# lfalive/fast-genomic-data-processing

Hardware: AMD Instinct MI355X
Metric: PairHMM GCUPS (higher is better)
Workload: dtype f32

## Files before the change

fast-genomic-data-processing_amd/csrc/mgx_pairhmm.hip:

```cpp
#include <hip/hip_runtime.h>

#include <algorithm>
#include <atomic>
#include <cerrno>
#include <cmath>
#include <cstdarg>
#include <cstdio>
#include <cstdlib>
#include <cstring>
#include <chrono>
#include <memory>
#include <mutex>
#include <new>
#include <thread>
#include <string>
#include <vector>

#include "../../include/mgx_pairhmm.h"
#include "mgx_common.h"
#include "mgx_tables.h"
#include "pairhmm_pack.h"
#include "pairhmm_kernels.hip.inc"

using mgx::set_error;

namespace {

constexpr int kNarrowMaxRPL = 8, kG8MaxRPL = 8, kG16MaxRPL = 12, kG64MinRPL = 4, kG64MaxRPL = 16;
constexpr int kMaxRowsG4 = 4 * kNarrowMaxRPL, kMaxRowsG8 = 8 * kG8MaxRPL;
constexpr int kMaxRowsG16 = 16 * kG16MaxRPL;
constexpr int kMaxRowsG64 = 64 * kG64MaxRPL;
constexpr int kMaxRowsStrip = 1 << 20;
constexpr int kStripMarkRPL = kG64MaxRPL + 1;
constexpr uint32_t kMaxLdsPerBlock = 64 * 1024;

struct Bin {
    int G = 0, RPL = 0;
    int Gd = 0, RPLd = 0;
    uint32_t job_begin = 0, job_count = 0;
    uint32_t max_h = 0;
    uint64_t cells = 0, alg_bytes = 0;
    uint32_t block = 256, lds_stride = 0, grid_f32 = 0, grid_f64 = 0, grid_f64_all = 0;
    bool strip = false;
};


struct Slab {
    uint8_t* dev = nullptr;
    uint8_t* pin = nullptr;
    size_t cap = 0, pin_cap = 0;
};
constexpr size_t kStageLimit = 256u << 20;
constexpr size_t kMaxEventSets = 64;
constexpr size_t kMinSlab = 1u << 20;
}

struct mgx_pairhmm {
    int device = 0;
    unsigned flags = 0;
    hipStream_t compute = nullptr, copy = nullptr, d2h = nullptr;
    static constexpr int kAux = 3;
    hipStream_t aux[kAux] = {nullptr, nullptr, nullptr};
    hipEvent_t ev_fork = nullptr, ev_join[kAux] = {nullptr, nullptr, nullptr};
    int n_streams = 1;
    float* d_ph2pr_f = nullptr; float* d_mm_f = nullptr; float* d_div3_f = nullptr; float* d_ratio_f = nullptr;
    double* d_ph2pr_d = nullptr; double* d_mm_d = nullptr; double* d_div3_d = nullptr; double* d_ratio_d = nullptr;
    float log10_initial_f = 0; double log10_initial_d = 0;
    int n_cu = 256;
    std::vector<Slab> free_slabs;
    void* d_strip = nullptr; size_t strip_cap = 0;
};

struct mgx_pairhmm_batch {
    uint64_t n_pairs = 0;
    std::vector<Bin> bins;
    Slab slab;
    size_t in_bytes = 0, o_out = 0, o_used = 0, result_bytes = 0;
    uint8_t *d_bases = nullptr, *d_qual = nullptr, *d_ins = nullptr, *d_del = nullptr,
            *d_gcp = nullptr, *d_hap = nullptr, *d_used = nullptr;
    Job* d_jobs = nullptr;
    uint32_t* d_rerun_list = nullptr;
    uint32_t* d_rerun_count = nullptr;
    double* d_out = nullptr;
    std::vector<Job> host_jobs;
    bool has_model = false;
    uint32_t n_reads = 0;
    uint64_t* d_read_len = nullptr;
    uint8_t* d_keep = nullptr;
    uint32_t *d_row_off = nullptr, *d_row_nh = nullptr;
    size_t o_keep = 0;
    double log10_rate = 0, max_err = 0;
    hipEvent_t uploaded = nullptr;
    std::vector<hipEvent_t> ev;
    std::vector<uint64_t> acct_cells, acct_bytes;
    std::vector<int8_t> acct_multi;
    uint32_t ev_sets = 0;
    uint32_t runs_timed = 0;
    hipEvent_t done = nullptr;
    bool ran = false;
    mgx_pairhmm_stats_t stats{};
};

namespace {

using BatchPtr = std::unique_ptr<mgx_pairhmm_batch, void (*)(mgx_pairhmm_batch*)>;
BatchPtr new_batch() {
    return BatchPtr(new (std::nothrow) mgx_pairhmm_batch, [](mgx_pairhmm_batch* p) { mgx_pairhmm_batch_destroy(nullptr, p); });
}

#define HIP_TRY(expr)                                                                      \
    do {                                                                                   \
        hipError_t e_ = (expr);                                                            \
        if (e_ != hipSuccess) {                                                            \
            set_error("%s failed: %s (%s:%d)", #expr, hipGetErrorString(e_), __FILE__,     \
                      __LINE__);                                                           \
            return -EIO;                                                                   \
        }                                                                                  \
    } while (0)

template <typename T>
int upload(T** dst, const void* src, size_t bytes, hipStream_t s) {
    *dst = nullptr;
    if (bytes == 0) bytes = 16;
    HIP_TRY(hipMalloc((void**)dst, bytes));
    if (src) HIP_TRY(hipMemcpyAsync(*dst, src, bytes, hipMemcpyHostToDevice, s));
    return 0;
}

inline void shape_of(uint32_t R, int* G, int* RPL) {
    static const int min_g = [] { const char* e = getenv("MGX_PAIRHMM_MIN_G"); const int v = e ? atoi(e) : 4; return v; }();
    const uint32_t g8_rows = (uint32_t)kMaxRowsG8;
    if (R <= (uint32_t)kMaxRowsG4 && min_g <= 4) { *G = 4; *RPL = (int)((R + 3) / 4); }
    else if (R <= g8_rows && min_g <= 8) { *G = 8; *RPL = (int)((R + 7) / 8); }
    else if (R <= (uint32_t)kMaxRowsG16) { *G = 16; *RPL = (int)((R + 15) / 16); }
    else if (R <= (uint32_t)kMaxRowsG64) { *G = 64; *RPL = std::max(kG64MinRPL, (int)((R + 63) / 64)); }
    else if (R <= (uint32_t)kMaxRowsStrip) { *G = 64; *RPL = kStripMarkRPL; }
    else { *G = 0; *RPL = 0; }
}
inline uint32_t lds_bytes(const Bin& bin, bool f32) {
    const uint32_t waves = bin.block / 64u, groups = bin.block / (uint32_t)(f32 ? bin.G : bin.Gd);
    const uint32_t etab = f32 ? (uint32_t)((bin.RPL + 1) / 2) * kNumCodes * 512u : 0u;
    return waves * etab + groups * bin.lds_stride;
}
constexpr int kBinG8 = kNarrowMaxRPL, kBinG16 = kBinG8 + kG8MaxRPL, kBinG64 = kBinG16 + kG16MaxRPL;
constexpr int kBinStrip = kBinG64 + (kG64MaxRPL - kG64MinRPL + 1);
constexpr int kBins = kBinStrip + 1;
inline int bin_index(int G, int RPL) {
    if (G == 64 && RPL == kStripMarkRPL) return kBinStrip;
    return G == 4 ? RPL - 1 : G == 8 ? kBinG8 + RPL - 1 : G == 16 ? kBinG16 + RPL - 1 : kBinG64 + RPL - kG64MinRPL;
}
inline void bin_shape(int k, Bin* b) {
    if (k == kBinStrip) { b->G = 64; b->RPL = kG64MaxRPL; b->Gd = 64; b->RPLd = kG64MaxRPL; b->strip = true; return; }
    if (k < kBinG8) { b->G = 4; b->RPL = k + 1; }
    else if (k < kBinG16) { b->G = 8; b->RPL = k - kBinG8 + 1; }
    else if (k < kBinG64) { b->G = 16; b->RPL = k - kBinG16 + 1; }
    else { b->G = 64; b->RPL = k - kBinG64 + kG64MinRPL; }
    if (b->G == 16 && b->RPL > 8) { b->Gd = 64; b->RPLd = (16 * b->RPL + 63) / 64; }
    else { b->Gd = b->G; b->RPLd = b->RPL; }
}
constexpr uint64_t kMergeBelow = 4096;

int finalize_bin(Bin& bin, int n_cu) {
    bin.lds_stride = (bin.max_h + 2u * (uint32_t)std::max(bin.G, bin.Gd) + 8u + 15u) & ~15u;
    bin.block = 64;
    if (const char* e = getenv("MGX_PAIRHMM_BLOCK")) { const int v = atoi(e); if (v == 64 || v == 128 || v == 256) bin.block = (uint32_t)v; }
    while (bin.block > 64u && lds_bytes(bin, true) > kMaxLdsPerBlock) bin.block /= 2;
    if (lds_bytes(bin, true) > 160u * 1024u) {
        set_error("haplotype of %u bases does not fit the LDS staging buffer", bin.max_h);
        return -E2BIG;
    }
    if (bin.strip) {
        bin.block = 64;
        bin.grid_f32 = bin.grid_f64 = bin.grid_f64_all = std::min<uint32_t>(bin.job_count, (uint32_t)n_cu * 4u);
        return 0;
    }
    const uint32_t gpb = bin.block / bin.G, gpbd = bin.block / bin.Gd;
    bin.grid_f32 = (bin.job_count + gpb - 1) / gpb;
    bin.grid_f64_all = (bin.job_count + gpbd - 1) / gpbd;
    bin.grid_f64 = std::min<uint32_t>(bin.grid_f64_all, (uint32_t)n_cu * 8u);
    return 0;
}
void merge_small_bins(uint64_t (&count)[kBins], int (&remap)[kBins]) {
    for (int k = 0; k < kBins; ++k) remap[k] = k;
    for (int k = 0; k + 1 < kBins; ++k) {
        if (k + 1 == kBinG8 || k + 1 == kBinG16 || k + 1 == kBinG64 || k + 1 == kBinStrip) continue;
        if (count[k] && count[k] < kMergeBelow) { count[k + 1] += count[k]; count[k] = 0; remap[k] = k + 1; }
    }
    for (int k = 0; k < kBins; ++k) { int t = k; while (remap[t] != t) t = remap[t]; remap[k] = t; }
}

inline size_t align_up(size_t x, size_t a = 256) { return (x + a - 1) / a * a; }

int acquire_slab(mgx_pairhmm* c, size_t bytes, size_t pin_bytes, Slab* out) {
    int best = -1;
    for (size_t i = 0; i < c->free_slabs.size(); ++i) {
        const Slab& f = c->free_slabs[i];
        if (f.cap >= bytes && f.pin_cap >= pin_bytes && (best < 0 || f.cap < c->free_slabs[best].cap)) best = (int)i;
    }
    if (best >= 0) { *out = c->free_slabs[best]; c->free_slabs.erase(c->free_slabs.begin() + best); return 0; }
    auto round = [](size_t want) {
        size_t cap = kMinSlab;
        while (cap < want) cap *= 2;
        if (cap > want + (want >> 2) && want > (64u << 20)) cap = align_up(want, 1u << 20);
        return cap;
    };
    Slab sl;
    sl.cap = round(bytes);
    HIP_TRY(hipMalloc((void**)&sl.dev, sl.cap));
    if (pin_bytes) {
        sl.pin_cap = std::min(sl.cap, round(pin_bytes));
        if (hipHostMalloc((void**)&sl.pin, sl.pin_cap, hipHostMallocDefault) != hipSuccess) {
            (void)hipFree(sl.dev);
            set_error("hipHostMalloc of %zu bytes failed", sl.pin_cap);
            return -ENOMEM;
        }
    }
    *out = sl;
    return 0;
}
void release_slab(mgx_pairhmm* c, Slab sl) {
    if (!sl.dev) return;
    if (c && c->free_slabs.size() < 16) { c->free_slabs.push_back(sl); return; }
    (void)hipFree(sl.dev);
    if (sl.pin) (void)hipHostFree(sl.pin);
}

using mgx::validate;

}

extern "C" {

int mgx_pairhmm_table_f32(int which, const float** out) {
    const auto& t = mgx::tables<float>();
    if (which == 0) { *out = t.ph2pr.data(); return mgx::kPh2prSize; }
    if (which == 1) { *out = t.mm.data(); return mgx::kMmSize; }
    return -EINVAL;
}
int mgx_pairhmm_table_f64(int which, const double** out) {
    const auto& t = mgx::tables<double>();
    if (which == 0) { *out = t.ph2pr.data(); return mgx::kPh2prSize; }
    if (which == 1) { *out = t.mm.data(); return mgx::kMmSize; }
    return -EINVAL;
}

int mgx_pairhmm_create(int device, unsigned flags, mgx_pairhmm_t** out) {
    if (!out) { set_error("out is NULL"); return -EINVAL; }
    *out = nullptr;
    int n_dev = 0;
    if (hipGetDeviceCount(&n_dev) != hipSuccess || n_dev <= 0) {
        set_error("no HIP device is visible (this library has no CPU fallback)");
        return -ENODEV;
    }
    if (device == -1) {
        static std::atomic<unsigned> next{0};
        device = (int)(next.fetch_add(1) % (unsigned)n_dev);
    }
    if (device < 0 || device >= n_dev) { set_error("device %d out of range (0..%d)", device, n_dev - 1); return -EINVAL; }
    HIP_TRY(hipSetDevice(device));
    std::unique_ptr<mgx_pairhmm> c(new (std::nothrow) mgx_pairhmm);
    if (!c) return -ENOMEM;
    c->device = device;
    c->flags = flags;
    hipDeviceProp_t prop;
    HIP_TRY(hipGetDeviceProperties(&prop, device));
    c->n_cu = prop.multiProcessorCount;
    {
        const unsigned pat = (flags >> 8) & 0xFFu;
        if (pat != 0 && pat != 0xFFu) {
            const int n_words = (c->n_cu + 31) / 32;
            std::vector<uint32_t> mask(n_words, 0);
            for (int cu = 0; cu < c->n_cu; ++cu) if ((pat >> (cu & 7)) & 1u) mask[cu >> 5] |= 1u << (cu & 31);
            HIP_TRY(hipExtStreamCreateWithCUMask(&c->compute, (uint32_t)n_words, mask.data()));
        } else {
            HIP_TRY(hipStreamCreateWithFlags(&c->compute, hipStreamNonBlocking));
        }
    }
    HIP_TRY(hipStreamCreateWithFlags(&c->copy, hipStreamNonBlocking));
    HIP_TRY(hipStreamCreateWithFlags(&c->d2h, hipStreamNonBlocking));
    {
        const unsigned pat = (flags >> 8) & 0xFFu;
        const char* e = getenv("MGX_PAIRHMM_STREAMS");
        c->n_streams = e ? std::max(1, std::min(1 + mgx_pairhmm::kAux, atoi(e))) : 1;
        if (pat != 0 && pat != 0xFFu) c->n_streams = 1;
        for (int a = 0; a + 1 < c->n_streams; ++a) {
            HIP_TRY(hipStreamCreateWithFlags(&c->aux[a], hipStreamNonBlocking));
            HIP_TRY(hipEventCreateWithFlags(&c->ev_join[a], hipEventDisableTiming));
        }
        HIP_TRY(hipEventCreateWithFlags(&c->ev_fork, hipEventDisableTiming));
    }
    const auto& tf = mgx::tables<float>();
    const auto& td = mgx::tables<double>();
    int rc;
    if ((rc = upload(&c->d_ph2pr_f, tf.ph2pr.data(), tf.ph2pr.size() * 4, c->compute))) return rc;
    if ((rc = upload(&c->d_mm_f, tf.mm.data(), tf.mm.size() * 4, c->compute))) return rc;
    if ((rc = upload(&c->d_ph2pr_d, td.ph2pr.data(), td.ph2pr.size() * 8, c->compute))) return rc;
    if ((rc = upload(&c->d_mm_d, td.mm.data(), td.mm.size() * 8, c->compute))) return rc;
    if ((rc = upload(&c->d_div3_f, tf.ph2pr_div3.data(), tf.ph2pr_div3.size() * 4, c->compute))) return rc;
    if ((rc = upload(&c->d_ratio_f, tf.gap_ratio.data(), tf.gap_ratio.size() * 4, c->compute))) return rc;
    if ((rc = upload(&c->d_div3_d, td.ph2pr_div3.data(), td.ph2pr_div3.size() * 8, c->compute))) return rc;
    if ((rc = upload(&c->d_ratio_d, td.gap_ratio.data(), td.gap_ratio.size() * 8, c->compute))) return rc;
    c->log10_initial_f = tf.log10_initial;
    c->log10_initial_d = td.log10_initial;
    HIP_TRY(hipStreamSynchronize(c->compute));
    *out = c.release();
    return 0;
}

void mgx_pairhmm_destroy(mgx_pairhmm_t* c) {
    if (!c) return;
    (void)hipSetDevice(c->device);
    (void)hipFree(c->d_ph2pr_f); (void)hipFree(c->d_mm_f);
    (void)hipFree(c->d_ph2pr_d); (void)hipFree(c->d_mm_d);
    (void)hipFree(c->d_div3_f); (void)hipFree(c->d_ratio_f); (void)hipFree(c->d_div3_d); (void)hipFree(c->d_ratio_d);
    for (auto& sl : c->free_slabs) { (void)hipFree(sl.dev); if (sl.pin) (void)hipHostFree(sl.pin); }
    (void)hipFree(c->d_strip);
    if (c->compute) (void)hipStreamDestroy(c->compute);
    if (c->copy) (void)hipStreamDestroy(c->copy);
    if (c->d2h) (void)hipStreamDestroy(c->d2h);
    for (int a = 0; a < mgx_pairhmm::kAux; ++a) { if (c->aux[a]) (void)hipStreamDestroy(c->aux[a]); if (c->ev_join[a]) (void)hipEventDestroy(c->ev_join[a]); }
    if (c->ev_fork) (void)hipEventDestroy(c->ev_fork);
    delete c;
}

void mgx_pairhmm_batch_destroy(mgx_pairhmm_t* c, mgx_pairhmm_batch_t* b) {
    if (!b) return;
    if (c) {
        (void)hipSetDevice(c->device);
        if (b->done) (void)hipEventSynchronize(b->done);
        else if (b->uploaded) (void)hipEventSynchronize(b->uploaded);
    }
    release_slab(c, b->slab);
    if (b->uploaded) (void)hipEventDestroy(b->uploaded);
    if (b->done) (void)hipEventDestroy(b->done);
    for (auto e : b->ev) (void)hipEventDestroy(e);
    delete b;
}

namespace {

struct SlabLayout {
    uint64_t n = 0, n_reads = 0, n_haps = 0, n_regions = 0, read_bytes = 0, hap_bytes = 0;
    bool cross = false, model = false;
    size_t rtab = 0, rreg = 0, rpre = 0, gtab = 0, htab = 0;
    size_t jobs = 0, bases = 0, qual = 0, ins = 0, del = 0, gcp = 0, hap = 0;
    size_t mapq = 0, rlen = 0, roff = 0, rnh = 0;
    size_t rlist = 0, rcount = 0;
    size_t pin_bytes = 0;
    bool staged = true;
};

int lay_out_slab(mgx_pairhmm* c, bool always_stage, SlabLayout* L, mgx_pairhmm_batch* b) {
    size_t off = 0;
    auto take = [&off](size_t bytes) { const size_t at = off; off = align_up(off + bytes); return at; };
    const uint64_t n = L->n, per_read = L->model ? L->n_reads : 0;
    if (L->cross) {
        L->rtab = take(L->n_reads * sizeof(SeqRef));
        L->rreg = take(L->n_reads * sizeof(uint32_t));
        L->rpre = take((L->n_reads + 1) * sizeof(uint32_t));
        L->gtab = take(L->n_regions * sizeof(RegionRef));
        L->htab = take(L->n_haps * sizeof(SeqRef));
    } else {
        L->jobs = take(n * sizeof(Job));
    }
    L->bases = take(L->read_bytes);
    L->qual = take(L->read_bytes);
    L->ins = take(L->read_bytes);
    L->del = take(L->read_bytes);
    L->gcp = take(L->read_bytes);
    L->hap = take(L->hap_bytes);
    L->mapq = take(per_read);
    L->rlen = take(per_read * sizeof(uint64_t));
    L->roff = take(per_read * sizeof(uint32_t));
    L->rnh = take(per_read * sizeof(uint32_t));
    b->in_bytes = off;
    b->o_out = take(n * sizeof(double));
    b->o_used = take(n);
    b->o_keep = take(per_read);
    b->result_bytes = off - b->o_out;
    L->pin_bytes = off;
    if (L->cross) L->jobs = take(n * sizeof(Job));
    L->rlist = take(2 * n * sizeof(uint32_t));
    L->rcount = take(64 * sizeof(uint32_t));
    L->staged = always_stage || L->pin_bytes <= kStageLimit;
    if (const int rc = acquire_slab(c, off, L->staged ? L->pin_bytes : 0, &b->slab)) return rc;
    uint8_t* dv = b->slab.dev;
    b->d_jobs = (Job*)(dv + L->jobs);
    b->d_bases = dv + L->bases; b->d_qual = dv + L->qual; b->d_ins = dv + L->ins; b->d_del = dv + L->del;
    b->d_gcp = dv + L->gcp; b->d_hap = dv + L->hap;
    b->d_out = (double*)(dv + b->o_out); b->d_used = dv + b->o_used;
    b->d_rerun_list = (uint32_t*)(dv + L->rlist); b->d_rerun_count = (uint32_t*)(dv + L->rcount);
    if (L->model) {
        b->d_read_len = (uint64_t*)(dv + L->rlen); b->d_keep = dv + b->o_keep;
        b->d_row_off = (uint32_t*)(dv + L->roff); b->d_row_nh = (uint32_t*)(dv + L->rnh);
    }
    return 0;
}

ReadModel make_read_model(const mgx_read_model_t& model) {
    ReadModel rm{};
    rm.rate_factor = model.pcr_rate_factor; rm.bq_threshold = model.base_quality_threshold;
    rm.constant_gcp = model.constant_gcp;
    for (int i = 0; i <= 20; ++i) {
        const double d = 40.0 - std::exp((double)i / ((double)std::max(rm.rate_factor, 1) * M_PI));
        const int v = (d > 0.0 ? (int)(d + 0.5) : (int)(d - 0.5)) + 1;
        rm.pcr_cache[i] = (uint8_t)(char)std::max(10, v);
    }
    return rm;
}

struct CrossRead { uint64_t off; uint32_t len, region; uint8_t bin; };
struct CrossPlan {
    uint64_t nr = 0, nh = 0, n = 0, read_bytes = 0, hap_bytes = 0;
    std::vector<CrossRead> reads;
    std::vector<RegionRef> regions;
    std::vector<SeqRef> haps;
    uint32_t max_h = 0;
    uint64_t reads_in[kBins] = {0}, rstart[kBins + 1] = {0}, jobs_in[kBins] = {0}, cells_in[kBins] = {0}, bytes_in[kBins] = {0};
};

int cross_totals(uint32_t n_regions, const mgx_pairhmm_input_t* regs, CrossPlan* p, std::vector<uint64_t>* out_base) {
    out_base->assign(n_regions + 1, 0);
    for (uint32_t g = 0; g < n_regions; ++g) {
        const mgx_pairhmm_input_t& in = regs[g];
        if (in.pair_read || in.pair_hap) { set_error("region %u: regions are given in the cross-product form (pair arrays NULL)", g); return -EINVAL; }
        p->nr += in.n_reads; p->nh += in.n_haps; p->n += in.n_reads * in.n_haps;
        if (in.n_reads) p->read_bytes += in.read_off[in.n_reads] - in.read_off[0];
        if (in.n_haps) p->hap_bytes += in.hap_off[in.n_haps] - in.hap_off[0];
        (*out_base)[g + 1] = p->n;
    }
    if (p->n > 0xFFFFFFF0ull || p->nr > 0xFFFFFFF0ull) { set_error("more than 2^32 test cases in one batch"); return -E2BIG; }
    return 0;
}

int cross_tables(uint32_t n_regions, const mgx_pairhmm_input_t* regs, const std::vector<uint64_t>& out_base, CrossPlan* p,
                 uint64_t (&count)[kBins]) {
    p->reads.resize(p->nr); p->regions.resize(n_regions); p->haps.resize(p->nh);
    uint64_t r_at = 0, h_at = 0, rb = 0, hb = 0;
    for (uint32_t g = 0; g < n_regions; ++g) {
        const mgx_pairhmm_input_t& in = regs[g];
        RegionRef& R = p->regions[g];
        R.hap_begin = (uint32_t)h_at; R.n_haps = (uint32_t)in.n_haps; R.read_base = (uint32_t)r_at; R.out_base = (uint32_t)out_base[g];
        for (uint64_t h = 0; h < in.n_haps; ++h) {
            const uint64_t H = in.hap_off[h + 1] - in.hap_off[h];
            if (H == 0) { set_error("region %u: haplotype %llu is empty", g, (unsigned long long)h); return -EINVAL; }
            if (H > 0x7FFFFFF0ull) { set_error("haplotype too long"); return -E2BIG; }
            p->haps[h_at + h] = SeqRef{hb + (in.hap_off[h] - in.hap_off[0]), (uint32_t)H, (uint32_t)h};
            p->max_h = std::max<uint32_t>(p->max_h, (uint32_t)H);
        }
        std::stable_sort(p->haps.begin() + h_at, p->haps.begin() + h_at + in.n_haps, [](const SeqRef& a, const SeqRef& b2) { return a.len > b2.len; });
        for (uint64_t r = 0; r < in.n_reads; ++r) {
            const uint64_t Rl = in.read_off[r + 1] - in.read_off[r];
            if (Rl == 0) { set_error("region %u: read %llu is empty", g, (unsigned long long)r); return -EINVAL; }
            int G, RPL;
            shape_of((uint32_t)std::min<uint64_t>(Rl, 0xFFFFFFFFull), &G, &RPL);
            if (G == 0) { set_error("region %u: read of %llu bases exceeds the %d-row limit", g, (unsigned long long)Rl, kMaxRowsStrip); return -E2BIG; }
            CrossRead& ri = p->reads[r_at + r];
            ri.off = rb + (in.read_off[r] - in.read_off[0]); ri.len = (uint32_t)Rl; ri.region = g; ri.bin = (uint8_t)bin_index(G, RPL);
            count[ri.bin] += in.n_haps;
        }
        if (in.n_reads) rb += in.read_off[in.n_reads] - in.read_off[0];
        if (in.n_haps) hb += in.hap_off[in.n_haps] - in.hap_off[0];
        r_at += in.n_reads; h_at += in.n_haps;
    }
    return 0;
}

void cross_bins(CrossPlan* p, uint64_t (&count)[kBins]) {
    int remap[kBins];
    merge_small_bins(count, remap);
    std::vector<uint64_t> sumH(p->regions.size(), 0);
    for (size_t g = 0; g < p->regions.size(); ++g)
        for (uint32_t h = 0; h < p->regions[g].n_haps; ++h) sumH[g] += p->haps[p->regions[g].hap_begin + h].len;
    for (CrossRead& ri : p->reads) {
        ri.bin = (uint8_t)remap[ri.bin];
        const RegionRef& R = p->regions[ri.region];
        p->reads_in[ri.bin]++; p->jobs_in[ri.bin] += R.n_haps; p->cells_in[ri.bin] += (uint64_t)ri.len * sumH[ri.region];
        p->bytes_in[ri.bin] += 5ull * ri.len * R.n_haps + sumH[ri.region] + 4ull * R.n_haps;
    }
    for (int k = 0; k < kBins; ++k) p->rstart[k + 1] = p->rstart[k] + p->reads_in[k];
}

void cross_stage(const CrossPlan& p, uint32_t n_regions, const mgx_pairhmm_input_t* regs, const SlabLayout& L, uint8_t* pin) {
    SeqRef* rtab = (SeqRef*)(pin + L.rtab);
    uint32_t* rreg = (uint32_t*)(pin + L.rreg);
    uint32_t* rpre = (uint32_t*)(pin + L.rpre);
    uint64_t cur[kBins];
    for (int k = 0; k < kBins; ++k) cur[k] = p.rstart[k];
    for (uint64_t r = 0; r < p.nr; ++r) {
        const CrossRead& ri = p.reads[r];
        const uint64_t at = cur[ri.bin]++;
        rtab[at] = SeqRef{ri.off, ri.len, (uint32_t)r};
        rreg[at] = ri.region;
    }
    uint32_t run = 0;
    for (uint64_t at = 0; at < p.nr; ++at) { rpre[at] = run; run += p.regions[rreg[at]].n_haps; }
    rpre[p.nr] = run;
    memcpy(pin + L.gtab, p.regions.data(), n_regions * sizeof(RegionRef));
    memcpy(pin + L.htab, p.haps.data(), p.nh * sizeof(SeqRef));
    size_t rb = 0, hb = 0;
    for (uint32_t g = 0; g < n_regions; ++g) {
        const mgx_pairhmm_input_t& in = regs[g];
        if (in.n_reads) {
            const uint64_t o0 = in.read_off[0], len = in.read_off[in.n_reads] - o0;
            memcpy(pin + L.bases + rb, in.bases + o0, len); memcpy(pin + L.qual + rb, in.qual + o0, len);
            memcpy(pin + L.ins + rb, in.ins + o0, len);     memcpy(pin + L.del + rb, in.del + o0, len);
            memcpy(pin + L.gcp + rb, in.gcp + o0, len);
            rb += len;
        }
        if (in.n_haps) {
            const uint64_t o0 = in.hap_off[0], len = in.hap_off[in.n_haps] - o0;
            memcpy(pin + L.hap + hb, in.hap_bases + o0, len);
            hb += len;
        }
    }
}

int cross_stage_model(uint32_t n_regions, const mgx_pairhmm_input_t* regs, const uint8_t* const* mapq,
                      const std::vector<uint64_t>& out_base, const SlabLayout& L, uint8_t* pin) {
    uint64_t* rlen = (uint64_t*)(pin + L.rlen);
    uint32_t* roff = (uint32_t*)(pin + L.roff);
    uint32_t* rnh = (uint32_t*)(pin + L.rnh);
    uint64_t r_at = 0;
    for (uint32_t g = 0; g < n_regions; ++g) {
        const mgx_pairhmm_input_t& in = regs[g];
        if (in.n_reads && !mapq[g]) { set_error("region %u: mapq is NULL", g); return -EINVAL; }
        for (uint64_t r = 0; r < in.n_reads; ++r) {
            rlen[r_at + r] = in.read_off[r + 1] - in.read_off[r];
            roff[r_at + r] = (uint32_t)(out_base[g] + r * in.n_haps);
            rnh[r_at + r] = (uint32_t)in.n_haps;
        }
        if (in.n_reads) memcpy(pin + L.mapq + r_at, mapq[g], in.n_reads);
        r_at += in.n_reads;
    }
    return 0;
}

int create_cross(mgx_pairhmm_t* c, uint32_t n_regions, const mgx_pairhmm_input_t* regs, mgx_pairhmm_batch* b,
                 std::vector<uint64_t>* out_base, const uint8_t* const* mapq = nullptr, const mgx_read_model_t* model = nullptr) {
    CrossPlan p;
    int rc;
    if ((rc = cross_totals(n_regions, regs, &p, out_base))) return rc;
    b->n_pairs = p.n;
    b->stats.n_pairs = p.n;
    if (p.n == 0) return 0;
    uint64_t count[kBins] = {0};
    if ((rc = cross_tables(n_regions, regs, *out_base, &p, count))) return rc;
    cross_bins(&p, count);
    SlabLayout L;
    L.n = p.n; L.n_reads = p.nr; L.n_haps = p.nh; L.n_regions = n_regions; L.read_bytes = p.read_bytes; L.hap_bytes = p.hap_bytes;
    L.cross = true; L.model = model != nullptr;
    if ((rc = lay_out_slab(c, true, &L, b))) return rc;
    uint8_t* dv = b->slab.dev; uint8_t* pin = b->slab.pin;
    cross_stage(p, n_regions, regs, L, pin);
    hipStream_t s = c->copy;
    if (model) {
        if ((rc = cross_stage_model(n_regions, regs, mapq, *out_base, L, pin))) return rc;
        b->has_model = true; b->n_reads = (uint32_t)p.nr;
        b->log10_rate = model->log10_mismapping_rate; b->max_err = model->max_error_per_base;
    }
    HIP_TRY(hipMemcpyAsync(dv, pin, b->in_bytes, hipMemcpyHostToDevice, s));
    if (model)
        hipLaunchKernelGGL(pairhmm_read_model, dim3((uint32_t)p.nr), dim3(128), 0, s, (const SeqRef*)(dv + L.rtab),
                           b->d_bases, b->d_qual, b->d_ins, b->d_del, b->d_gcp, (const uint8_t*)(dv + L.mapq), make_read_model(*model));
    uint64_t job_begin = 0;
    for (int k = 0; k < kBins; ++k) {
        if (!p.reads_in[k]) continue;
        Bin bin;
        bin_shape(k, &bin);
        bin.job_begin = (uint32_t)job_begin;
        bin.job_count = (uint32_t)p.jobs_in[k];
        bin.max_h = p.max_h;
        bin.cells = p.cells_in[k];
        bin.alg_bytes = p.bytes_in[k];
        if ((rc = finalize_bin(bin, c->n_cu))) return rc;
        b->stats.cells += bin.cells; b->stats.alg_bytes += bin.alg_bytes;
        b->bins.push_back(bin);
        job_begin += bin.job_count;
    }
    hipLaunchKernelGGL(pairhmm_make_jobs_multi, dim3((uint32_t)((p.n + 255) / 256)), dim3(256), 0, s, (const SeqRef*)(dv + L.rtab),
                       (const uint32_t*)(dv + L.rreg), (const uint32_t*)(dv + L.rpre), (uint32_t)p.nr, (const RegionRef*)(dv + L.gtab),
                       (const SeqRef*)(dv + L.htab), (uint32_t)p.n, b->d_jobs);
    HIP_TRY(hipGetLastError());
    HIP_TRY(hipEventCreateWithFlags(&b->uploaded, hipEventDisableTiming));
    HIP_TRY(hipEventRecord(b->uploaded, s));
    return 0;
}

int upload_pairs(mgx_pairhmm_t* c, const mgx_pairhmm_input_t* in, const mgx::PackPlan* plan, const SlabLayout& L, const Job* jobs,
                 mgx_pairhmm_batch* b) {
    const uint64_t read_bytes = L.read_bytes, hap_bytes = L.hap_bytes;
    uint8_t* dv = b->slab.dev;
    hipStream_t s = c->copy;
    if (L.staged) {
        uint8_t* pin = b->slab.pin;
        if (plan) {
            mgx::pack_copy(in, *plan, pin + L.bases, pin + L.qual, pin + L.ins, pin + L.del, pin + L.gcp, pin + L.hap);
        } else if (read_bytes + hap_bytes < (32u << 20)) {
            memcpy(pin + L.bases, in->bases, read_bytes); memcpy(pin + L.qual, in->qual, read_bytes);
            memcpy(pin + L.ins, in->ins, read_bytes);     memcpy(pin + L.del, in->del, read_bytes);
            memcpy(pin + L.gcp, in->gcp, read_bytes);     memcpy(pin + L.hap, in->hap_bases, hap_bytes);
        } else {
            const void* src[6] = {in->bases, in->qual, in->ins, in->del, in->gcp, in->hap_bases};
            uint8_t* dst[6] = {pin + L.bases, pin + L.qual, pin + L.ins, pin + L.del, pin + L.gcp, pin + L.hap};
            const size_t len[6] = {(size_t)read_bytes, (size_t)read_bytes, (size_t)read_bytes, (size_t)read_bytes, (size_t)read_bytes, (size_t)hap_bytes};
            std::thread th[6];
            for (int k = 0; k < 6; ++k) th[k] = std::thread([=] { memcpy(dst[k], src[k], len[k]); });
            for (auto& t : th) t.join();
        }
        HIP_TRY(hipMemcpyAsync(dv, pin, b->in_bytes, hipMemcpyHostToDevice, s));
    } else {
        HIP_TRY(hipMemcpyAsync(b->d_jobs, jobs, L.n * sizeof(Job), hipMemcpyHostToDevice, s));
        HIP_TRY(hipMemcpyAsync(b->d_bases, in->bases, read_bytes, hipMemcpyHostToDevice, s));
        HIP_TRY(hipMemcpyAsync(b->d_qual, in->qual, read_bytes, hipMemcpyHostToDevice, s));
        HIP_TRY(hipMemcpyAsync(b->d_ins, in->ins, read_bytes, hipMemcpyHostToDevice, s));
        HIP_TRY(hipMemcpyAsync(b->d_del, in->del, read_bytes, hipMemcpyHostToDevice, s));
        HIP_TRY(hipMemcpyAsync(b->d_gcp, in->gcp, read_bytes, hipMemcpyHostToDevice, s));
        HIP_TRY(hipMemcpyAsync(b->d_hap, in->hap_bases, hap_bytes, hipMemcpyHostToDevice, s));
        HIP_TRY(hipStreamSynchronize(s));
        b->host_jobs.clear(); b->host_jobs.shrink_to_fit();
    }
    HIP_TRY(hipEventCreateWithFlags(&b->uploaded, hipEventDisableTiming));
    HIP_TRY(hipEventRecord(b->uploaded, s));
    return 0;
}

int create_pairs(mgx_pairhmm_t* c, const mgx_pairhmm_input_t* in, const mgx::PackPlan* plan, mgx_pairhmm_batch* b) {
    const uint64_t n = plan ? plan->hi - plan->lo : in->n_pairs;
    const uint32_t* pr = plan ? plan->pair_read.data() : in->pair_read;
    const uint32_t* ph = plan ? plan->pair_hap.data() : in->pair_hap;
    const uint64_t* roff = plan ? plan->roff.data() : in->read_off;
    const uint64_t* hoff = plan ? plan->hoff.data() : in->hap_off;
    const uint64_t n_reads = plan ? plan->lread.size() : in->n_reads, n_haps = plan ? plan->lhap.size() : in->n_haps;
    int rc;
    b->n_pairs = n;
    b->stats.n_pairs = n;

    std::vector<uint32_t> bin_of(n);
    uint64_t count[kBins] = {0};
    uint32_t max_h = 0;
    for (uint64_t i = 0; i < n; ++i) {
        const uint32_t r = pr[i], h = ph[i];
        if (r >= n_reads || h >= n_haps) { set_error("test case %llu: index out of range", (unsigned long long)i); return -EINVAL; }
        const uint64_t R = roff[r + 1] - roff[r];
        const uint64_t H = hoff[h + 1] - hoff[h];
        if (R == 0 || H == 0) { set_error("test case %llu: empty read or haplotype", (unsigned long long)i); return -EINVAL; }
        int G, RPL;
        shape_of((uint32_t)std::min<uint64_t>(R, 0xFFFFFFFFull), &G, &RPL);
        if (G == 0) { set_error("test case %llu: read of %llu bases exceeds the %d-row limit", (unsigned long long)i, (unsigned long long)R, kMaxRowsStrip); return -E2BIG; }
        if (H > 0x7FFFFFF0ull) { set_error("haplotype too long"); return -E2BIG; }
        const int bi = bin_index(G, RPL);
        bin_of[i] = (uint32_t)bi;
        count[bi]++;
        max_h = std::max<uint32_t>(max_h, (uint32_t)H);
        b->stats.cells += R * H;
        b->stats.alg_bytes += 5 * R + H + 4;
    }
    {
        int remap[kBins];
        merge_small_bins(count, remap);
        for (uint64_t i = 0; i < n; ++i) bin_of[i] = (uint32_t)remap[bin_of[i]];
    }
    SlabLayout L;
    L.n = n; L.n_reads = n_reads; L.n_haps = n_haps; L.read_bytes = roff[n_reads]; L.hap_bytes = hoff[n_haps];
    if ((rc = lay_out_slab(c, plan != nullptr, &L, b))) return rc;
    if (!L.staged) b->host_jobs.resize(n);
    Job* jobs = L.staged ? (Job*)(b->slab.pin + L.jobs) : b->host_jobs.data();
    {
        std::vector<uint64_t> bin_start(kBins + 1, 0);
        for (int k = 0; k < kBins; ++k) bin_start[k + 1] = bin_start[k] + count[k];
        std::vector<std::vector<uint32_t>> hist(kBins);
        for (int k = 0; k < kBins; ++k) if (count[k]) hist[k].assign((size_t)max_h + 2, 0);
        for (uint64_t i = 0; i < n; ++i) {
            const uint32_t h = ph[i];
            const uint32_t H = (uint32_t)(hoff[h + 1] - hoff[h]);
            hist[bin_of[i]][(max_h - H) + 1]++;
        }
        for (int k = 0; k < kBins; ++k)
            for (size_t x = 1; x < hist[k].size(); ++x) hist[k][x] += hist[k][x - 1];
        for (uint64_t i = 0; i < n; ++i) {
            const uint32_t r = pr[i], h = ph[i];
            const uint32_t R = (uint32_t)(roff[r + 1] - roff[r]);
            const uint32_t H = (uint32_t)(hoff[h + 1] - hoff[h]);
            const int k = (int)bin_of[i];
            Job& jb = jobs[bin_start[k] + hist[k][max_h - H]++];
            jb.read_off = roff[r]; jb.hap_off = hoff[h];
            jb.R = R; jb.H = H; jb.pair = (uint32_t)i; jb.pad_ = 0;
        }
        for (int k = 0; k < kBins; ++k) {
            if (!count[k]) continue;
            Bin bin;
            bin_shape(k, &bin);
            bin.job_begin = (uint32_t)bin_start[k];
            bin.job_count = (uint32_t)count[k];
            for (uint64_t q = bin_start[k]; q < bin_start[k + 1]; ++q) {
                bin.max_h = std::max(bin.max_h, jobs[q].H);
                bin.cells += (uint64_t)jobs[q].R * jobs[q].H;
                bin.alg_bytes += 5ull * jobs[q].R + jobs[q].H + 4;
            }
            if ((rc = finalize_bin(bin, c->n_cu))) return rc;
            b->bins.push_back(bin);
        }
    }
    return upload_pairs(c, in, plan, L, jobs, b);
}

}

int mgx_pairhmm_batch_create(mgx_pairhmm_t* c, const mgx_pairhmm_input_t* in,
                             mgx_pairhmm_batch_t** out) {
    if (!c || !out) { set_error("ctx/out is NULL"); return -EINVAL; }
    *out = nullptr;
    int rc = validate(in);
    if (rc) return rc;
    HIP_TRY(hipSetDevice(c->device));
    BatchPtr b = new_batch();
    if (!b) return -ENOMEM;
    std::vector<uint64_t> base;
    if (!in->pair_read && !in->pair_hap && in->n_reads && in->n_haps) rc = create_cross(c, 1, in, b.get(), &base);
    else rc = create_pairs(c, in, nullptr, b.get());
    if (rc) return rc;
    *out = b.release();
    return 0;
}

namespace {

constexpr int kSharedCount = 63;
constexpr int kExactCount = 62;

inline bool is_narrow(const Bin& bn) { return bn.G <= 16 && bn.G * bn.RPL <= 16 * kNarrowMaxRPL; }

struct Run {
    mgx_pairhmm* c = nullptr;
    mgx_pairhmm_batch* b = nullptr;
    hipStream_t s = nullptr;
    bool timing = false, force_f64 = false;
    hipEvent_t* ev = nullptr;
    int n_str = 1;
    KernelArgs base{};
    std::vector<char> in_multi;
    size_t first_narrow = 0;
    uint32_t n_narrow_jobs = 0, narrow_max_h = 0, narrow_rows = 0;
};

int ensure_strip_scratch(mgx_pairhmm* c, size_t bytes) {
    if (bytes <= c->strip_cap) return 0;
    HIP_TRY(hipStreamSynchronize(c->compute));
    (void)hipFree(c->d_strip); c->d_strip = nullptr; c->strip_cap = 0;
    HIP_TRY(hipMalloc(&c->d_strip, bytes));
    c->strip_cap = bytes;
    return 0;
}

int pick_event_set(Run& r) {
    mgx_pairhmm_batch* b = r.b;
    if (!r.timing) return 0;
    if (b->ev.empty()) {
        const size_t per = b->bins.size() * 4;
        b->ev_sets = (uint32_t)std::max<size_t>(1, std::min<size_t>(kMaxEventSets, 1024 / per));
        b->ev.resize(per * b->ev_sets);
        for (auto& e : b->ev) HIP_TRY(hipEventCreate(&e));
    }
    r.ev = b->ev.data() + (size_t)(b->runs_timed % b->ev_sets) * b->bins.size() * 4;
    return 0;
}

int begin_run(Run& r) {
    mgx_pairhmm* c = r.c; mgx_pairhmm_batch* b = r.b;
    if (b->uploaded) HIP_TRY(hipStreamWaitEvent(r.s, b->uploaded, 0));
    HIP_TRY(hipMemsetAsync(b->d_rerun_count, 0, 64 * sizeof(uint32_t), r.s));
    HIP_TRY(hipMemsetAsync(b->d_used, 0, b->n_pairs, r.s));
    r.n_str = (int)std::min<size_t>((size_t)c->n_streams, b->bins.size());
    if (r.n_str > 1) {
        HIP_TRY(hipEventRecord(c->ev_fork, r.s));
        for (int q = 0; q + 1 < r.n_str; ++q) HIP_TRY(hipStreamWaitEvent(c->aux[q], c->ev_fork, 0));
    }
    KernelArgs& base = r.base;
    base.jobs = b->d_jobs;
    base.bases = b->d_bases; base.qual = b->d_qual; base.ins = b->d_ins; base.del = b->d_del;
    base.gcp = b->d_gcp; base.hap_bases = b->d_hap;
    base.out_log10 = b->d_out; base.used_f64 = b->d_used;
    base.log10_initial_f = c->log10_initial_f;
    base.log10_initial_d = c->log10_initial_d;
    return 0;
}

void survey_narrow(Run& r) {
    const std::vector<Bin>& bins = r.b->bins;
    r.first_narrow = bins.size();
    for (size_t k = 0; k < bins.size(); ++k) {
        const Bin& bn = bins[k];
        if (!is_narrow(bn)) continue;
        if (r.first_narrow == bins.size()) r.first_narrow = k;
        r.n_narrow_jobs = std::max(r.n_narrow_jobs, bn.job_begin + bn.job_count);
        r.narrow_max_h = std::max(r.narrow_max_h, bn.max_h);
        r.narrow_rows = std::max(r.narrow_rows, (uint32_t)(bn.G * bn.RPL));
    }
}

int launch_f64(const Run& r, KernelArgs a, int Gd, int RPLd, uint32_t grid, uint32_t block, uint32_t lds, hipStream_t sk) {
    const mgx_pairhmm* c = r.c;
    a.ph2pr = c->d_ph2pr_d; a.mm = c->d_mm_d; a.ph2pr_div3 = c->d_div3_d; a.gap_ratio = c->d_ratio_d;
    a.rerun_list = r.b->d_rerun_list + r.b->n_pairs; a.rerun_count = r.b->d_rerun_count + kExactCount;
    KernelFn f = a.strip_scratch ? (KernelFn)pairhmm_fwd_strip<double> : pick_kernel<double>(Gd, RPLd);
    if (!f) { set_error("no fp64 kernel for G=%d RPL=%d", Gd, RPLd); return -ENOSYS; }
    hipLaunchKernelGGL(f, dim3(grid), dim3(block), lds, sk, a);
    return 0;
}

int launch_multi(Run& r, int gset, std::vector<size_t>& set) {
    mgx_pairhmm* c = r.c; mgx_pairhmm_batch* b = r.b;
    std::stable_sort(set.begin(), set.end(), [&](size_t x, size_t y) {
        const Bin &bx = b->bins[x], &by = b->bins[y];
        return bx.RPL != by.RPL ? bx.RPL > by.RPL : bx.G > by.G;
    });
    MultiArgs m{};
    m.a = r.base;
    m.a.rerun_list = b->d_rerun_list; m.a.rerun_count = b->d_rerun_count + kSharedCount;
    m.a.job_list = nullptr; m.a.n_dyn = nullptr;
    m.a.ph2pr = c->d_ph2pr_f; m.a.mm = c->d_mm_f; m.a.ph2pr_div3 = c->d_div3_f; m.a.gap_ratio = c->d_ratio_f;
    m.n_bins = (uint32_t)set.size();
    uint32_t blocks = 0, lds = 0;
    size_t book = set[0];
    uint64_t cells = 0, bytes = 0;
    for (size_t q = 0; q < set.size(); ++q) {
        const Bin& bn = b->bins[set[q]];
        m.block_first[q] = blocks; blocks += bn.grid_f32;
        m.job_first[q] = bn.job_begin; m.job_count[q] = bn.job_count; m.lds_stride[q] = bn.lds_stride;
        m.G[q] = (uint8_t)bn.G; m.RPL[q] = (uint8_t)bn.RPL;
        lds = std::max(lds, lds_bytes(bn, true));
        if (bn.cells > b->bins[book].cells) book = set[q];
        cells += bn.cells; bytes += bn.alg_bytes;
        r.in_multi[set[q]] = 1;
        b->acct_cells[set[q]] = 0; b->acct_bytes[set[q]] = 0;
    }
    m.block_first[set.size()] = blocks;
    b->acct_cells[book] = cells; b->acct_bytes[book] = bytes; b->acct_multi[book] = (int8_t)(1 + gset);
    if (r.timing) for (size_t q : set) if (q != book) { HIP_TRY(hipEventRecord(r.ev[4 * q + 0], r.s)); HIP_TRY(hipEventRecord(r.ev[4 * q + 1], r.s)); }
    if (r.timing) HIP_TRY(hipEventRecord(r.ev[4 * book + 0], r.s));
    if (gset == 0) hipLaunchKernelGGL(pairhmm_fwd_multi<0>, dim3(blocks), dim3(64), lds, r.s, m);
    else           hipLaunchKernelGGL(pairhmm_fwd_multi<1>, dim3(blocks), dim3(64), lds, r.s, m);
    if (r.timing) HIP_TRY(hipEventRecord(r.ev[4 * book + 1], r.s));
    return 0;
}

int launch_multi_classes(Run& r) {
    mgx_pairhmm_batch* b = r.b;
    static const bool multi_ok = [] { const char* e = getenv("MGX_PAIRHMM_MULTI"); return !e || atoi(e) != 0; }();
    const uint32_t multi_below = (uint32_t)r.c->n_cu * 64u;
    r.in_multi.assign(b->bins.size(), 0);
    b->acct_cells.assign(b->bins.size(), 0); b->acct_bytes.assign(b->bins.size(), 0); b->acct_multi.assign(b->bins.size(), 0);
    for (size_t k = 0; k < b->bins.size(); ++k) { b->acct_cells[k] = b->bins[k].cells; b->acct_bytes[k] = b->bins[k].alg_bytes; }
    if (!multi_ok || r.force_f64) return 0;
    for (int gset = 0; gset < 2; ++gset) {
        std::vector<size_t> set;
        for (size_t k = 0; k < b->bins.size(); ++k) {
            const Bin& bn = b->bins[k];
            if (is_narrow(bn) && bn.RPL <= kNarrowMaxRPL && bn.block == 64 && bn.grid_f32 < multi_below && (gset == 0 ? bn.G == 16 : bn.G < 16)) set.push_back(k);
        }
        if (set.size() < 2 || set.size() > (size_t)kMultiBins) continue;
        if (const int rc = launch_multi(r, gset, set)) return rc;
    }
    return 0;
}

int launch_class(Run& r, size_t k, hipStream_t sk) {
    mgx_pairhmm* c = r.c; mgx_pairhmm_batch* b = r.b;
    hipEvent_t* ev = r.ev;
    const Bin& bin = b->bins[k];
    const bool shared = is_narrow(bin) && !r.force_f64;
    KernelArgs a = r.base;
    if (bin.strip) {
        a.strip_stride = (bin.max_h + 63u) & ~63u;
        if (const int rc = ensure_strip_scratch(c, (size_t)bin.grid_f32 * 6u * a.strip_stride * sizeof(double))) return rc;
        a.strip_scratch = c->d_strip;
    }
    a.rerun_list = shared ? b->d_rerun_list : b->d_rerun_list + bin.job_begin;
    a.rerun_count = b->d_rerun_count + (shared ? kSharedCount : (int)k);
    a.lds_stride = bin.lds_stride;
    a.job_first = bin.job_begin;
    if (!r.force_f64 && !r.in_multi[k]) {
        a.job_list = nullptr; a.n_dyn = nullptr; a.n_static = bin.job_count;
        a.ph2pr = c->d_ph2pr_f; a.mm = c->d_mm_f; a.ph2pr_div3 = c->d_div3_f; a.gap_ratio = c->d_ratio_f;
        KernelFn f = bin.strip ? (KernelFn)pairhmm_fwd_strip<float> : pick_kernel<float>(bin.G, bin.RPL);
        if (!f) { set_error("no fp32 kernel for G=%d RPL=%d", bin.G, bin.RPL); return -ENOSYS; }
        if (r.timing) HIP_TRY(hipEventRecord(ev[4 * k + 0], sk));
        hipLaunchKernelGGL(f, dim3(bin.grid_f32), dim3(bin.block), lds_bytes(bin, true), sk, a);
        if (r.timing) HIP_TRY(hipEventRecord(ev[4 * k + 1], sk));
    }
    const bool books_shared = shared && k == r.first_narrow;
    if (r.timing && !books_shared) HIP_TRY(hipEventRecord(ev[4 * k + 2], sk));
    if (!shared) {
        if (r.force_f64) { a.job_list = nullptr; a.n_dyn = nullptr; a.n_static = bin.job_count; }
        else { a.job_list = a.rerun_list; a.n_dyn = a.rerun_count; a.n_static = 0; }
        const int rc = launch_f64(r, a, bin.Gd, bin.RPLd, r.force_f64 ? bin.grid_f64_all : bin.grid_f64, bin.block, lds_bytes(bin, false), sk);
        if (rc) return rc;
    }
    if (r.timing && !books_shared) HIP_TRY(hipEventRecord(ev[4 * k + 3], sk));
    return 0;
}

int launch_classes(Run& r) {
    mgx_pairhmm* c = r.c; mgx_pairhmm_batch* b = r.b;
    std::vector<size_t> order(b->bins.size());
    for (size_t k = 0; k < order.size(); ++k) order[k] = k;
    std::stable_sort(order.begin(), order.end(), [&](size_t x, size_t y) { return b->bins[x].cells > b->bins[y].cells; });
    for (size_t at = 0; at < order.size(); ++at) {
        hipStream_t sk = (int)(at % (size_t)r.n_str) == 0 ? r.s : c->aux[at % (size_t)r.n_str - 1];
        if (const int rc = launch_class(r, order[at], sk)) return rc;
    }
    for (int q = 0; q + 1 < r.n_str; ++q) {
        HIP_TRY(hipEventRecord(c->ev_join[q], c->aux[q]));
        HIP_TRY(hipStreamWaitEvent(r.s, c->ev_join[q], 0));
    }
    return 0;
}

int launch_shared_f64(Run& r) {
    if (!r.n_narrow_jobs || r.force_f64) return 0;
    KernelArgs a = r.base;
    a.job_list = r.b->d_rerun_list; a.n_dyn = r.b->d_rerun_count + kSharedCount; a.n_static = 0; a.job_first = 0;
    a.lds_stride = (r.narrow_max_h + 2u * 16u + 8u + 15u) & ~15u;
    const int RPLd = (int)((r.narrow_rows + 15) / 16);
    const uint32_t grid = std::min<uint32_t>((r.n_narrow_jobs + 3) / 4, (uint32_t)r.c->n_cu * 8u);
    if (r.timing) HIP_TRY(hipEventRecord(r.ev[4 * r.first_narrow + 2], r.s));
    if (const int rc = launch_f64(r, a, 16, RPLd, grid, 64, 4u * a.lds_stride, r.s)) return rc;
    if (r.timing) HIP_TRY(hipEventRecord(r.ev[4 * r.first_narrow + 3], r.s));
    return 0;
}

int launch_exact(Run& r) {
    mgx_pairhmm* c = r.c; mgx_pairhmm_batch* b = r.b;
    uint32_t max_h = 0;
    for (const Bin& bn : b->bins) max_h = std::max(max_h, bn.max_h);
    KernelArgs a = r.base;
    a.ph2pr = c->d_ph2pr_d; a.mm = c->d_mm_d; a.ph2pr_div3 = c->d_div3_d; a.gap_ratio = c->d_ratio_d;
    a.job_list = b->d_rerun_list + b->n_pairs; a.n_dyn = b->d_rerun_count + kExactCount; a.n_static = 0; a.job_first = 0;
    a.rerun_list = nullptr; a.rerun_count = nullptr;
    a.lds_stride = (max_h + 2u * 64u + 8u + 15u) & ~15u;
    a.strip_stride = (max_h + 63u) & ~63u;
    const size_t per_wg = 6u * (size_t)a.strip_stride * sizeof(double);
    const uint32_t grid = (uint32_t)std::max<size_t>(1, std::min<size_t>({(size_t)b->n_pairs, (size_t)c->n_cu * 2u, (size_t)(256u << 20) / per_wg}));
    if (const int rc = ensure_strip_scratch(c, (size_t)grid * per_wg)) return rc;
    a.strip_scratch = c->d_strip;
    hipLaunchKernelGGL(pairhmm_fwd_exact, dim3(grid), dim3(64), a.lds_stride, r.s, a);
    return 0;
}

void launch_epilogue(Run& r) {
    const mgx_pairhmm_batch* b = r.b;
    if (!b->has_model) return;
    hipLaunchKernelGGL(pairhmm_normalize_filter_rows, dim3((b->n_reads + 3) / 4), dim3(256), 0, r.s, b->d_out, b->d_read_len,
                       b->d_row_off, b->d_row_nh, b->n_reads, b->log10_rate, b->max_err, b->d_keep);
}

}

int mgx_pairhmm_batch_run(mgx_pairhmm_t* c, mgx_pairhmm_batch_t* b) {
    if (!c || !b) { set_error("ctx/batch is NULL"); return -EINVAL; }
    HIP_TRY(hipSetDevice(c->device));
    if (b->n_pairs == 0) { b->ran = true; return 0; }
    Run r;
    r.c = c; r.b = b; r.s = c->compute;
    r.timing = (c->flags & MGX_PAIRHMM_TIMING) != 0 && !b->bins.empty();
    r.force_f64 = (c->flags & MGX_PAIRHMM_FORCE_DOUBLE) != 0;
    int rc;
    if ((rc = pick_event_set(r))) return rc;
    if ((rc = begin_run(r))) return rc;
    survey_narrow(r);
    if ((rc = launch_multi_classes(r))) return rc;
    if ((rc = launch_classes(r))) return rc;
    if ((rc = launch_shared_f64(r))) return rc;
    if ((rc = launch_exact(r))) return rc;
    launch_epilogue(r);
    HIP_TRY(hipGetLastError());
    if (r.timing) b->runs_timed++;
    if (!b->done) HIP_TRY(hipEventCreateWithFlags(&b->done, hipEventDisableTiming));
    HIP_TRY(hipEventRecord(b->done, r.s));
    b->ran = true;
    return 0;
}

int mgx_pairhmm_sync(mgx_pairhmm_t* c) {
    if (!c) { set_error("ctx is NULL"); return -EINVAL; }
    HIP_TRY(hipSetDevice(c->device));
    HIP_TRY(hipStreamSynchronize(c->compute));
    return 0;
}

int mgx_pairhmm_batch_stats(mgx_pairhmm_t* c, mgx_pairhmm_batch_t* b, mgx_pairhmm_stats_t* out) {
    if (!c || !b || !out) { set_error("NULL argument"); return -EINVAL; }
    HIP_TRY(hipSetDevice(c->device));
    HIP_TRY(hipStreamSynchronize(c->compute));
    mgx_pairhmm_stats_t st = b->stats;
    const bool force_f64 = (c->flags & MGX_PAIRHMM_FORCE_DOUBLE) != 0;
    st.n_launches_f32 = force_f64 ? 0 : (uint32_t)b->bins.size();
    st.n_launches_f64 = (uint32_t)b->bins.size();
    st.n_rerun_f64 = 0;
    if (b->ran && b->n_pairs) {
        std::vector<uint32_t> cnt(64);
        HIP_TRY(hipMemcpy(cnt.data(), b->d_rerun_count, 64 * sizeof(uint32_t), hipMemcpyDeviceToHost));
        for (size_t k = 0; k < b->bins.size(); ++k) st.n_rerun_f64 += force_f64 ? b->bins[k].job_count : cnt[k];
        if (!force_f64) st.n_rerun_f64 += cnt[63];
        st.n_exact = cnt[62];
    }
    st.ms_f32 = st.ms_f64 = st.ms_f32_dominant = 0;
    st.dominant_cells = st.dominant_alg_bytes = 0;
    st.dominant_kernel[0] = 0;
    st.n_runs_timed = 0;
    if ((c->flags & MGX_PAIRHMM_TIMING) && b->ran && !b->ev.empty() && b->runs_timed) {
        const uint32_t n_sets = std::min(b->runs_timed, b->ev_sets);
        const bool acct = b->acct_cells.size() == b->bins.size();
        auto cells_of = [&](size_t k) { return acct ? b->acct_cells[k] : b->bins[k].cells; };
        size_t dom = 0;
        for (size_t k = 0; k < b->bins.size(); ++k) if (cells_of(k) >= cells_of(dom)) dom = k;
        double f32 = 0, f64 = 0, domms = 0;
        for (uint32_t q = 0; q < n_sets; ++q) {
            const uint32_t set = (b->runs_timed - 1 - q) % b->ev_sets;
            hipEvent_t* ev = b->ev.data() + (size_t)set * b->bins.size() * 4;
            for (size_t k = 0; k < b->bins.size(); ++k) {
                float ms = 0;
                if (!force_f64) {
                    HIP_TRY(hipEventElapsedTime(&ms, ev[4 * k + 0], ev[4 * k + 1]));
                    f32 += ms;
                    if (k == dom) domms += ms;
                }
                float ms2 = 0;
                HIP_TRY(hipEventElapsedTime(&ms2, ev[4 * k + 2], ev[4 * k + 3]));
                f64 += ms2;
            }
        }
        st.n_runs_timed = n_sets;
        st.ms_f32 = (float)(f32 / n_sets); st.ms_f64 = (float)(f64 / n_sets);
        if (!force_f64) {
            st.ms_f32_dominant = (float)(domms / n_sets);
            st.dominant_cells = cells_of(dom);
            st.dominant_alg_bytes = acct ? b->acct_bytes[dom] : b->bins[dom].alg_bytes;
            if (acct && b->acct_multi[dom]) snprintf(st.dominant_kernel, sizeof st.dominant_kernel, "pairhmm_fwd_multi<%d>", b->acct_multi[dom] - 1);
            else snprintf(st.dominant_kernel, sizeof st.dominant_kernel, "pairhmm_fwd<float, %d, %d>", b->bins[dom].G, b->bins[dom].RPL);
        }
        b->runs_timed = 0;
    }
    *out = st;
    return 0;
}

namespace {
int fetch_results(mgx_pairhmm_t* c, mgx_pairhmm_batch_t* b, size_t bytes) {
    hipStream_t s = c->d2h;
    if (b->done) HIP_TRY(hipStreamWaitEvent(s, b->done, 0));
    HIP_TRY(hipMemcpyAsync(b->slab.pin + b->o_out, b->d_out, bytes, hipMemcpyDeviceToHost, s));
    HIP_TRY(hipStreamSynchronize(s));
    return 0;
}

void scatter_region_results(const mgx_pairhmm_batch* b, const std::vector<uint64_t>& base, const mgx_pairhmm_input_t* regions,
                            uint32_t g0, uint32_t g1, double* const* out, uint8_t* const* keep) {
    const double* all = (const double*)(b->slab.pin + b->o_out);
    const uint8_t* kept = b->slab.pin + b->o_keep;
    uint64_t r_at = 0;
    for (uint32_t g = g0; g < g1; ++g) {
        const uint64_t a = base[g - g0], e = base[g - g0 + 1];
        if (e > a) memcpy(out[g], all + a, (e - a) * sizeof(double));
        if (keep && keep[g] && e > a) memcpy(keep[g], kept + r_at, regions[g].n_reads);
        r_at += regions[g].n_reads;
    }
}

void cut_regions(const mgx_pairhmm_input_t* regions, uint32_t n_regions, uint64_t limit, std::vector<uint32_t>* cut) {
    cut->assign(1, 0);
    uint64_t in_run = 0;
    for (uint32_t g = 0; g < n_regions; ++g) {
        const uint64_t n = regions[g].n_reads * regions[g].n_haps;
        if (in_run && in_run + n > limit) { cut->push_back(g); in_run = 0; }
        in_run += n;
    }
    if (n_regions) cut->push_back(n_regions);
}
}

int mgx_pairhmm_batch_results(mgx_pairhmm_t* c, mgx_pairhmm_batch_t* b, double* out_log10,
                              uint8_t* used_f64) {
    if (!c || !b) { set_error("ctx/batch is NULL"); return -EINVAL; }
    if (!b->ran) { set_error("batch has not been run"); return -EINVAL; }
    HIP_TRY(hipSetDevice(c->device));
    if (b->n_pairs == 0) return 0;
    if (!out_log10) { set_error("out_log10 is NULL"); return -EINVAL; }
    if (b->slab.pin) {
        const int rc = fetch_results(c, b, used_f64 ? b->o_used + b->n_pairs - b->o_out : b->n_pairs * sizeof(double));
        if (rc) return rc;
        memcpy(out_log10, b->slab.pin + b->o_out, b->n_pairs * sizeof(double));
        if (used_f64) memcpy(used_f64, b->slab.pin + b->o_used, b->n_pairs);
        return 0;
    }
    hipStream_t s = c->d2h;
    if (b->done) HIP_TRY(hipStreamWaitEvent(s, b->done, 0));
    HIP_TRY(hipMemcpyAsync(out_log10, b->d_out, b->n_pairs * sizeof(double), hipMemcpyDeviceToHost, s));
    if (used_f64) HIP_TRY(hipMemcpyAsync(used_f64, b->d_used, b->n_pairs, hipMemcpyDeviceToHost, s));
    HIP_TRY(hipStreamSynchronize(s));
    return 0;
}

void mgx_read_model_defaults(mgx_read_model_t* m) {
    if (!m) return;
    m->pcr_rate_factor = 3;
    m->base_quality_threshold = 18;
    m->constant_gcp = 10;
    m->log10_mismapping_rate = -4.5;
    m->max_error_per_base = 0.02;
}

int mgx_pairhmm_compute(mgx_pairhmm_t* c, const mgx_pairhmm_input_t* in, double* out_log10) {
    mgx_pairhmm_batch_t* b = nullptr;
    int rc = mgx_pairhmm_batch_create(c, in, &b);
    if (rc) return rc;
    rc = mgx_pairhmm_batch_run(c, b);
    if (!rc) rc = mgx_pairhmm_batch_results(c, b, out_log10, nullptr);
    mgx_pairhmm_batch_destroy(c, b);
    return rc;
}

int mgx_pairhmm_regions(mgx_pairhmm_t* c, uint32_t n_regions, const mgx_pairhmm_input_t* regions, const uint8_t* const* mapq,
                        const mgx_read_model_t* model, double* const* out_log10, uint8_t* const* out_keep) {
    if (!c || !model || (n_regions && (!regions || !mapq || !out_log10))) { set_error("NULL argument"); return -EINVAL; }
    if (n_regions == 0) return 0;
    int rc;
    for (uint32_t g = 0; g < n_regions; ++g) {
        if ((rc = validate(&regions[g]))) return rc;
        if (regions[g].n_reads * regions[g].n_haps && !out_log10[g]) { set_error("region %u: output pointer is NULL", g); return -EINVAL; }
    }
    HIP_TRY(hipSetDevice(c->device));
    BatchPtr b = new_batch();
    if (!b) return -ENOMEM;
    std::vector<uint64_t> base;
    if ((rc = create_cross(c, n_regions, regions, b.get(), &base, mapq, model))) return rc;
    if (b->n_pairs == 0) return 0;
    mgx_pairhmm_batch* raw = b.release();
    rc = mgx_pairhmm_batch_run(c, raw);
    if (!rc) {
        rc = [&]() -> int {
            HIP_TRY(hipMemcpyAsync(raw->slab.pin + raw->o_out, raw->d_out, raw->result_bytes, hipMemcpyDeviceToHost, c->compute));
            HIP_TRY(hipStreamSynchronize(c->compute));
            return 0;
        }();
        if (!rc) scatter_region_results(raw, base, regions, 0, n_regions, out_log10, out_keep);
    }
    mgx_pairhmm_batch_destroy(c, raw);
    return rc;
}

int mgx_pairhmm_region(mgx_pairhmm_t* c, const mgx_pairhmm_input_t* in, const uint8_t* mapq,
                       const mgx_read_model_t* model, double* out_log10, uint8_t* out_keep) {
    if (!c || !in || !mapq || !model || !out_log10) { set_error("NULL argument"); return -EINVAL; }
    if (in->pair_read || in->pair_hap) { set_error("mgx_pairhmm_region takes the cross-product form (pair arrays NULL)"); return -EINVAL; }
    int rc = validate(in);
    if (rc) return rc;
    if (in->n_reads == 0 || in->n_haps == 0) return 0;
    return mgx_pairhmm_regions(c, 1, in, &mapq, model, &out_log10, out_keep ? &out_keep : nullptr);
}

int mgx_pairhmm_compute_regions(mgx_pairhmm_t* c, uint32_t n_regions, const mgx_pairhmm_input_t* regions, double* const* out_log10) {
    if (!c || (n_regions && (!regions || !out_log10))) { set_error("NULL argument"); return -EINVAL; }
    if (n_regions == 0) return 0;
    int rc;
    for (uint32_t g = 0; g < n_regions; ++g) {
        if ((rc = validate(&regions[g]))) return rc;
        if (regions[g].n_reads * regions[g].n_haps && !out_log10[g]) { set_error("region %u: output pointer is NULL", g); return -EINVAL; }
    }
    HIP_TRY(hipSetDevice(c->device));
    uint64_t kChunkPairs = 3u << 16;
    {
        uint64_t total = 0;
        for (uint32_t g = 0; g < n_regions; ++g) total += regions[g].n_reads * regions[g].n_haps;
        kChunkPairs = std::min<uint64_t>(6u << 16, std::max<uint64_t>(kChunkPairs, total / 6));
    }
    if (const char* e = getenv("MGX_PAIRHMM_REGION_CHUNK")) { const long long v = atoll(e); if (v > 0) kChunkPairs = (uint64_t)v; }
    std::vector<uint32_t> cut;
    cut_regions(regions, n_regions, kChunkPairs, &cut);
    struct InFlight { mgx_pairhmm_batch_t* b = nullptr; uint32_t g0 = 0, g1 = 0; std::vector<uint64_t> base; };
    InFlight fl[2];
    auto retire = [&](InFlight& f) -> int {
        if (!f.b) return 0;
        const int r = fetch_results(c, f.b, f.b->n_pairs * sizeof(double));
        if (!r) scatter_region_results(f.b, f.base, regions, f.g0, f.g1, out_log10, nullptr);
        mgx_pairhmm_batch_destroy(c, f.b);
        f.b = nullptr;
        return r;
    };
    rc = 0;
    for (size_t k = 0; k + 1 < cut.size() && !rc; ++k) {
        InFlight& f = fl[k & 1];
        rc = retire(f);
        if (rc) break;
        BatchPtr b = new_batch();
        if (!b) { rc = -ENOMEM; break; }
        f.g0 = cut[k]; f.g1 = cut[k + 1];
        if ((rc = create_cross(c, f.g1 - f.g0, regions + f.g0, b.get(), &f.base))) break;
        if (b->n_pairs == 0) continue;
        f.b = b.release();
        rc = mgx_pairhmm_batch_run(c, f.b);
    }
    for (int q = 0; q < 2; ++q) { const int r = retire(fl[(cut.size() - 1 + q) & 1]); if (!rc) rc = r; }
    return rc;
}

struct mgx_pairhmm_queue {
    struct Lane {
        mgx_pairhmm* ctx = nullptr;
        uint32_t dev_slot = 0;
        double pack_s = 0, wait_s = 0;
        uint64_t batches = 0, bytes_h2d = 0, bytes_d2h = 0, cells = 0;
    };
    std::vector<Lane> lanes;
    uint32_t n_devices = 1, depth = 2, batch_pairs = 65536;
    mgx_pairhmm_queue_stats_t stats{};
};

namespace {

struct QueueRun {
    const mgx_pairhmm_input_t* in = nullptr;
    uint64_t lo = 0, hi = 0, n_batches = 0;
    double* out = nullptr;
    uint8_t* used = nullptr;
    const mgx_pairhmm_input_t* regions = nullptr;
    double* const* region_out = nullptr;
    std::vector<uint32_t> chunk;
    std::atomic<uint64_t> next{0};
    std::atomic<int> failed{0};
    std::mutex err_mu;
    int rc = 0;
    std::string err;
    void fail(int code) {
        std::lock_guard<std::mutex> g(err_mu);
        if (!rc) { rc = code; err = mgx_last_error(); }
        failed.store(1);
    }
};

double now_s() { return std::chrono::duration<double>(std::chrono::steady_clock::now().time_since_epoch()).count(); }

void queue_lane(mgx_pairhmm_queue* q, mgx_pairhmm_queue::Lane* ln, QueueRun* run) {
    struct Slot { mgx_pairhmm_batch* b = nullptr; uint64_t lo = 0; uint32_t g0 = 0, g1 = 0; std::vector<uint64_t> base; };
    std::vector<Slot> slots(q->depth);
    mgx::PackPlan plan;
    mgx_pairhmm* c = ln->ctx;
    if (hipSetDevice(c->device) != hipSuccess) { set_error("hipSetDevice(%d) failed", c->device); run->fail(-EIO); return; }
    auto retire = [&](Slot& sl) {
        if (!sl.b) return;
        const double t0 = now_s();
        if (!run->failed.load()) {
            int rc = 0;
            if (run->regions) {
                rc = fetch_results(c, sl.b, sl.b->n_pairs * sizeof(double));
                if (!rc) scatter_region_results(sl.b, sl.base, run->regions, sl.g0, sl.g1, run->region_out, nullptr);
                ln->bytes_d2h += sl.b->n_pairs * 8;
            } else {
                const uint64_t at = sl.lo - run->lo;
                rc = mgx_pairhmm_batch_results(c, sl.b, run->out + at, run->used ? run->used + at : nullptr);
                ln->bytes_d2h += sl.b->n_pairs * (run->used ? 9 : 8);
            }
            if (rc) run->fail(rc);
        }
        mgx_pairhmm_batch_destroy(c, sl.b);
        sl.b = nullptr;
        ln->wait_s += now_s() - t0;
    };
    size_t turn = 0;
    while (!run->failed.load()) {
        const uint64_t k = run->next.fetch_add(1);
        if (k >= run->n_batches) break;
        Slot& sl = slots[turn++ % slots.size()];
        retire(sl);
        if (run->failed.load()) break;
        const double t0 = now_s();
        BatchPtr b = new_batch();
        int rc = b ? 0 : -ENOMEM;
        if (!rc && run->regions) {
            sl.g0 = run->chunk[k]; sl.g1 = run->chunk[k + 1];
            rc = create_cross(c, sl.g1 - sl.g0, run->regions + sl.g0, b.get(), &sl.base);
        } else if (!rc) {
            sl.lo = run->lo + k * q->batch_pairs;
            const uint64_t hi = std::min(run->hi, sl.lo + q->batch_pairs);
            const uint64_t bad = mgx::pack_plan(run->in, sl.lo, hi, &plan);
            if (bad) { set_error("test case %llu: index out of range", (unsigned long long)(sl.lo + bad - 1)); run->fail(-EINVAL); break; }
            rc = create_pairs(c, run->in, &plan, b.get());
        }
        ln->pack_s += now_s() - t0;
        if (!rc && b->n_pairs) rc = mgx_pairhmm_batch_run(c, b.get());
        if (rc) { run->fail(rc); break; }
        if (!b->n_pairs) continue;
        ln->batches++; ln->bytes_h2d += b->in_bytes; ln->cells += b->stats.cells;
        sl.b = b.release();
    }
    for (size_t j = 0; j < slots.size(); ++j) retire(slots[(turn + j) % slots.size()]);
}

int queue_execute(mgx_pairhmm_queue* q, QueueRun& run, uint64_t n_pairs) {
    for (auto& ln : q->lanes) { ln.pack_s = ln.wait_s = 0; ln.batches = ln.bytes_h2d = ln.bytes_d2h = ln.cells = 0; }
    const double t0 = now_s();
    const size_t n_thr = (size_t)std::min<uint64_t>(q->lanes.size(), run.n_batches);
    std::vector<std::thread> th;
    for (size_t i = 1; i < n_thr; ++i) th.emplace_back(queue_lane, q, &q->lanes[i], &run);
    queue_lane(q, &q->lanes[0], &run);
    for (auto& t : th) t.join();
    q->stats.seconds = now_s() - t0;
    q->stats.n_pairs = n_pairs;
    q->stats.n_batches = run.n_batches;
    for (auto& ln : q->lanes) {
        q->stats.cells += ln.cells; q->stats.bytes_h2d += ln.bytes_h2d; q->stats.bytes_d2h += ln.bytes_d2h;
        q->stats.pack_seconds += ln.pack_s; q->stats.wait_seconds += ln.wait_s;
        q->stats.batches_per_device[ln.dev_slot] += ln.batches;
    }
    if (run.rc) { set_error("%s", run.err.c_str()); return run.rc; }
    return 0;
}

}

int mgx_pairhmm_queue_create(const mgx_pairhmm_queue_config_t* cfg, mgx_pairhmm_queue_t** out) {
    if (!out) { set_error("out is NULL"); return -EINVAL; }
    *out = nullptr;
    mgx_pairhmm_queue_config_t d{};
    if (cfg) d = *cfg;
    const int dev0 = 0;
    const uint32_t n_dev = d.n_devices && d.devices ? d.n_devices : 1;
    if (n_dev > 16) { set_error("at most 16 devices per queue"); return -EINVAL; }
    const uint32_t lanes = d.lanes_per_device ? d.lanes_per_device : 4;
    if (lanes > 32) { set_error("at most 32 lanes per device"); return -EINVAL; }
    std::unique_ptr<mgx_pairhmm_queue> q(new (std::nothrow) mgx_pairhmm_queue);
    if (!q) return -ENOMEM;
    q->n_devices = n_dev;
    q->depth = d.depth ? std::min<uint32_t>(d.depth, 8) : 2;
    q->batch_pairs = d.batch_pairs ? d.batch_pairs : 65536;
    for (uint32_t v = 0; v < n_dev; ++v)
        for (uint32_t l = 0; l < lanes; ++l) {
            mgx_pairhmm_queue::Lane ln;
            ln.dev_slot = v;
            const int rc = mgx_pairhmm_create(d.n_devices && d.devices ? d.devices[v] : dev0, d.flags, &ln.ctx);
            if (rc) { for (auto& x : q->lanes) mgx_pairhmm_destroy(x.ctx); return rc; }
            q->lanes.push_back(ln);
        }
    *out = q.release();
    return 0;
}

void mgx_pairhmm_queue_destroy(mgx_pairhmm_queue_t* q) {
    if (!q) return;
    for (auto& ln : q->lanes) mgx_pairhmm_destroy(ln.ctx);
    delete q;
}

int mgx_pairhmm_queue_run_range(mgx_pairhmm_queue_t* q, const mgx_pairhmm_input_t* in, uint64_t pair_begin, uint64_t pair_end,
                                double* out_log10, uint8_t* used_f64) {
    if (!q) { set_error("queue is NULL"); return -EINVAL; }
    int rc = validate(in);
    if (rc) return rc;
    const uint64_t total = mgx::pack_n_pairs(in);
    if (pair_begin > pair_end || pair_end > total) { set_error("test-case range [%llu, %llu) outside the stream of %llu", (unsigned long long)pair_begin, (unsigned long long)pair_end, (unsigned long long)total); return -EINVAL; }
    q->stats = mgx_pairhmm_queue_stats_t{};
    q->stats.n_lanes = (uint32_t)q->lanes.size();
    if (pair_begin == pair_end) return 0;
    if (!out_log10) { set_error("out_log10 is NULL"); return -EINVAL; }
    QueueRun run;
    run.in = in; run.lo = pair_begin; run.hi = pair_end; run.out = out_log10; run.used = used_f64;
    run.n_batches = (pair_end - pair_begin + q->batch_pairs - 1) / q->batch_pairs;
    return queue_execute(q, run, pair_end - pair_begin);
}

int mgx_pairhmm_queue_run_regions(mgx_pairhmm_queue_t* q, uint32_t n_regions, const mgx_pairhmm_input_t* regions, double* const* out_log10) {
    if (!q || (n_regions && (!regions || !out_log10))) { set_error("NULL argument"); return -EINVAL; }
    q->stats = mgx_pairhmm_queue_stats_t{};
    q->stats.n_lanes = (uint32_t)q->lanes.size();
    QueueRun run;
    run.regions = regions; run.region_out = out_log10;
    uint64_t total = 0;
    for (uint32_t g = 0; g < n_regions; ++g) {
        int rc = validate(&regions[g]);
        if (rc) return rc;
        if (regions[g].pair_read || regions[g].pair_hap) { set_error("region %u: regions are given in the cross-product form (pair arrays NULL)", g); return -EINVAL; }
        const uint64_t n = regions[g].n_reads * regions[g].n_haps;
        if (n && !out_log10[g]) { set_error("region %u: output pointer is NULL", g); return -EINVAL; }
        total += n;
    }
    cut_regions(regions, n_regions, q->batch_pairs, &run.chunk);
    run.n_batches = run.chunk.size() - 1;
    if (total == 0) return 0;
    return queue_execute(q, run, total);
}

int mgx_pairhmm_queue_run(mgx_pairhmm_queue_t* q, const mgx_pairhmm_input_t* in, double* out_log10, uint8_t* used_f64) {
    if (!in) { set_error("input is NULL"); return -EINVAL; }
    return mgx_pairhmm_queue_run_range(q, in, 0, mgx::pack_n_pairs(in), out_log10, used_f64);
}

int mgx_pairhmm_queue_stats(mgx_pairhmm_queue_t* q, mgx_pairhmm_queue_stats_t* out) {
    if (!q || !out) { set_error("NULL argument"); return -EINVAL; }
    *out = q->stats;
    return 0;
}

}
```

fast-genomic-data-processing_amd/csrc/pairhmm_kernels.hip.inc:

```

#include <type_traits>

namespace {

struct Job {
    uint64_t read_off;
    uint64_t hap_off;
    uint32_t R;
    uint32_t H;
    uint32_t pair;
    uint32_t pad_;
};
static_assert(sizeof(Job) == 32, "Job is 32 bytes");

struct KernelArgs {
    const Job* jobs;
    const uint32_t* job_list;
    const uint32_t* n_dyn;
    uint32_t n_static;
    uint32_t job_first;
    const uint8_t* bases;
    const uint8_t* qual;
    const uint8_t* ins;
    const uint8_t* del;
    const uint8_t* gcp;
    const uint8_t* hap_bases;
    const void* ph2pr;
    const void* mm;
    const void* ph2pr_div3;
    const void* gap_ratio;
    double* out_log10;
    uint8_t* used_f64;
    uint32_t* rerun_list;
    uint32_t* rerun_count;
    uint32_t lds_stride;
    void* strip_scratch;
    uint32_t strip_stride;
    float log10_initial_f;
    double log10_initial_d;
};

constexpr double kExactBelow = 1e-280;
constexpr int kCodeN = 4;
constexpr int kCodePad = 7;

__device__ __forceinline__ int base_code(int b) {
    int c = 0;
    c = (b == 'C') ? 1 : c;
    c = (b == 'T') ? 2 : c;
    c = (b == 'G') ? 3 : c;
    c = (b == 'N') ? kCodeN : c;
    return c;
}

__device__ __forceinline__ uint32_t base_code4(uint32_t w) {
    const uint32_t sel = (w >> 1) & 0x07070707u;
    const uint32_t code = __builtin_amdgcn_perm(0x04000000u, 0x03020100u, sel);
    const uint32_t want = __builtin_amdgcn_perm(0x4E000000u, 0x47544341u, sel);
    const uint32_t diff = want ^ w;
    const uint32_t nz = (((diff & 0x7F7F7F7Fu) + 0x7F7F7F7Fu) | diff) & 0x80808080u;
    const uint32_t ok = ((nz ^ 0x80808080u) >> 7) * 0xFFu;
    return code & ok;
}

template <int G> constexpr int lane_stride() { return G < 16 ? 16 / G : 1; }

template <int G>
__device__ __forceinline__ int dpp_shr1(int old, int v) {
    if constexpr (G == 64)
        return __builtin_amdgcn_update_dpp(old, v, 0x138 , 0xf, 0xf, false);
    else
        return __builtin_amdgcn_update_dpp(old, v, 0x110 + lane_stride<G>() , 0xf, 0xf, false);
}
template <int G>
__device__ __forceinline__ float shr1(float old, float v) {
    return __builtin_bit_cast(float, dpp_shr1<G>(__builtin_bit_cast(int, old), __builtin_bit_cast(int, v)));
}
template <int G>
__device__ __forceinline__ double shr1(double old, double v) {
    long long o = __builtin_bit_cast(long long, old), x = __builtin_bit_cast(long long, v);
    unsigned lo = (unsigned)dpp_shr1<G>((int)(unsigned)o, (int)(unsigned)x);
    unsigned hi = (unsigned)dpp_shr1<G>((int)(unsigned)(o >> 32), (int)(unsigned)(x >> 32));
    return __builtin_bit_cast(double, ((long long)hi << 32) | (long long)lo);
}

template <int G, typename T>
__device__ __forceinline__ T shr1_down(T v) {
    const int lane = (int)(threadIdx.x & 63);
    constexpr int S = lane_stride<G>();
    const int j = G < 16 ? (lane & 15) / S : lane % G;
    const int src = (j == G - 1) ? lane : lane + S;
    return __shfl(v, src, 64);
}

__device__ __forceinline__ float fma_(float a, float b, float c) { return __builtin_fmaf(a, b, c); }
__device__ __forceinline__ double fma_(double a, double b, double c) { return __builtin_fma(a, b, c); }

template <typename T> struct Prec;
template <> struct Prec<float> {
    static __device__ __forceinline__ float initial() { return 0x1p120f; }
};
template <> struct Prec<double> {
    static __device__ __forceinline__ double initial() { return 0x1p1020; }
};

#ifndef MGX_PAIRHMM_CODES
#define MGX_PAIRHMM_CODES 5
#endif
constexpr int kNumCodes = MGX_PAIRHMM_CODES;
template <int RPL> constexpr int etab_bytes_per_wave() { return ((RPL + 1) / 2) * kNumCodes * 64 * 8; }

template <typename T, int G, int RPL, bool STRIP = false, bool EXACT = false>
__device__ __forceinline__ void pairhmm_body(const KernelArgs& a, uint8_t* smem, const uint32_t block, const uint32_t n_blocks) {
    constexpr int GPW = 64 / G;
    constexpr bool kETab = (sizeof(T) == 4);
    constexpr bool kSix = (sizeof(T) == 4) && !EXACT;
    constexpr int RP2 = (RPL + 1) / 2;
    constexpr int S = lane_stride<G>();
    const int gpb = (int)blockDim.x / G;
    const int tid = (int)threadIdx.x;
    const int lane = tid & 63;
    const int wave = tid >> 6;
    const int j = G < 16 ? (lane & 15) / S : lane % G;
    const int grp = wave * GPW + (G < 16 ? (lane >> 4) * S + (lane & 15) % S : lane / G);
    const int n_waves = (int)blockDim.x >> 6;
    uint8_t* etab = smem + (kETab ? (size_t)wave * etab_bytes_per_wave<RPL>() : 0);
    uint8_t* hapbuf = smem + (kETab ? (size_t)n_waves * etab_bytes_per_wave<RPL>() : 0) +
                      (size_t)grp * a.lds_stride;
    const T* __restrict__ ph2pr = (const T*)a.ph2pr;
    const T* __restrict__ mm = (const T*)a.mm;
    const T* __restrict__ ph2pr_div3 = (const T*)a.ph2pr_div3;
    const T* __restrict__ gap_ratio = (const T*)a.gap_ratio;
    const uint32_t n_jobs = a.n_dyn ? *a.n_dyn : a.n_static;

    for (uint32_t base = block * (uint32_t)gpb; base < n_jobs; base += n_blocks * (uint32_t)gpb) {
        const uint32_t slot = base + (uint32_t)grp;
        const bool live = slot < n_jobs;
        uint32_t job_idx = 0;
        Job job;
        job.read_off = 0; job.hap_off = 0; job.R = 0; job.H = 0; job.pair = 0; job.pad_ = 0;
        if (live) {
            job_idx = a.job_list ? a.job_list[slot] : a.job_first + slot;
            job = a.jobs[job_idx];
        }
        const int R = (int)job.R, H = (int)job.H;
        constexpr int kStripRows = G * RPL;
        const int n_strips = STRIP ? (R > kStripRows ? (R + kStripRows - 1) / kStripRows : 1) : 1;
        const int first_rows = R - (n_strips - 1) * kStripRows;

        __syncthreads();
        bool hap_n = false;
        {
            const uint8_t* hp = a.hap_bases + job.hap_off;
            const int n_words = (int)a.lds_stride >> 2;
            uint32_t* hb32 = reinterpret_cast<uint32_t*>(hapbuf);
            for (int w = j; w < n_words; w += G) {
                const int c0 = 4 * w - G;
                uint32_t packed;
                if (live && c0 >= 0 && c0 + 4 <= H) {
                    uint32_t raw;
                    __builtin_memcpy(&raw, hp + c0, 4);
                    packed = base_code4(raw);
                } else {
                    packed = 0;
#pragma unroll
                    for (int t = 0; t < 4; ++t) {
                        const int c = c0 + t;
                        const int code = (live && c >= 0 && c < H) ? base_code(hp[c]) : (kNumCodes > 4 ? kCodeN : 0);
                        packed |= (uint32_t)code << (8 * t);
                    }
                }
                if constexpr (kETab && kNumCodes == 4) {
                    const uint32_t x = packed ^ (0x01010101u * (uint32_t)kCodeN);
                    hap_n |= ((x - 0x01010101u) & ~x & 0x80808080u) != 0;
                    packed &= 0x03030303u;
                }
                hb32[w] = packed;
            }
        }
        bool group_hap_n = false;
        if constexpr (kETab && kNumCodes == 4) {
            uint64_t gmask;
            if constexpr (G == 64) gmask = ~0ull;
            else if constexpr (G == 16) gmask = 0xFFFFull << (lane & 48);
            else gmask = (uint64_t)((G == 8 ? 0x5555u : 0x1111u) << ((lane & 15) % S)) << (lane & 48);
            group_hap_n = (__ballot((int)hap_n) & gmask) != 0;
        }

        T sumM = 0, sumX = 0;
        bool zero_gap = false;
        if constexpr (STRIP) {
            for (int rr = lane; rr < R; rr += 64) zero_gap |= (a.gcp[job.read_off + (uint64_t)rr] & 127) == 0;
        }
        int nl = 0;
        T* const bnd = STRIP ? reinterpret_cast<T*>(a.strip_scratch) + (size_t)block * 6u * a.strip_stride : nullptr;
      for (int strip = 0; strip < n_strips; ++strip) {
        const int rows_here = (STRIP && strip > 0) ? kStripRows : first_rows;
        const int row_base = (STRIP && strip > 0) ? first_rows + (strip - 1) * kStripRows : 0;
        const bool last_strip = strip == n_strips - 1;
        nl = (rows_here + RPL - 1) / RPL;
        const int top_clones = nl * RPL - rows_here;
        volatile T* const bcur = STRIP ? bnd + (size_t)(strip & 1) * 3u * a.strip_stride : nullptr;
        const volatile T* const bprev = STRIP ? bnd + (size_t)((strip & 1) ^ 1) * 3u * a.strip_stride : nullptr;
        if (STRIP && strip > 0) __syncthreads();

        T k0[RPL], k1[RPL], k2[RPL], k3[RPL], k4[RPL], eM[RPL], eX[RPL];
        int rb[RPL];
        T pm[RPL], px[RPL], py[RPL];
        bool clone[RPL];
        T ratio[RPL];
        const T init_y = Prec<T>::initial() / (T)(H > 0 ? H : 1);
#pragma unroll
        for (int s = 0; s < RPL; ++s) {
            const int rho = j * RPL + s - top_clones;
            k0[s] = 0; k1[s] = 0; k2[s] = 0; k3[s] = 0; k4[s] = 0; eM[s] = 0; eX[s] = 0;
            rb[s] = 0; pm[s] = 0; px[s] = 0; py[s] = 0; clone[s] = false; ratio[s] = 0;
            if (live && j < nl) {
                if (rho < 0) {
                    clone[s] = true;
                    k3[s] = 1;
                    py[s] = init_y;
                } else {
                    const uint64_t o = job.read_off + (uint64_t)(row_base + rho);
                    const int qi = a.ins[o] & 127, qd = a.del[o] & 127, qc = a.gcp[o] & 127;
                    const int qq = a.qual[o] & 127;
                    const int mn = qi <= qd ? qi : qd, mx = qi <= qd ? qd : qi;
                    k0[s] = mm[((mx * (mx + 1)) >> 1) + mn];
                    k3[s] = ph2pr[qc];
                    k1[s] = (T)1.0 - ph2pr[qc];
                    k2[s] = ph2pr[qi];
                    k4[s] = ph2pr[qd];
                    zero_gap |= (qc == 0);
                    const T distm = ph2pr[qq];
                    eM[s] = (T)1.0 - distm;
                    const int code = base_code(a.bases[o]);
                    eX[s] = (code == kCodeN) ? eM[s] : ph2pr_div3[qq];
                    ratio[s] = gap_ratio[qc];
                    rb[s] = code;
                }
            }
        }
        if constexpr (kETab) {
            float* et = reinterpret_cast<float*>(etab) + lane * 2;
#pragma unroll
            for (int s = 0; s < RPL; ++s)
#pragma unroll
                for (int code = 0; code < kNumCodes; ++code)
                    et[((s >> 1) * kNumCodes + code) * 128 + (s & 1)] =
                        (code == rb[s] || code == kCodeN) ? eM[s] : eX[s];
        }
        __syncthreads();

        const int nsteps_g = live ? (H + nl - 1) : 0;
        int nmax = nsteps_g, nmin = live ? nsteps_g : 0x7fffffff;
        if constexpr (GPW > 1) {
#pragma unroll
            for (int off = 1; off < 64; off <<= 1) {
                if (off >= S && off < (G < 16 ? 16 : G)) continue;
                const int o1 = __shfl_xor(nmax, off, 64), o2 = __shfl_xor(nmin, off, 64);
                nmax = o1 > nmax ? o1 : nmax;
                nmin = o2 < nmin ? o2 : nmin;
            }
        }
        nmax = __builtin_amdgcn_readfirstlane(nmax);
        nmin = __builtin_amdgcn_readfirstlane(nmin);
        if (nmin > nmax) nmin = nmax;

        const uint8_t* hp_lane = hapbuf + (G - j);
        const uint8_t* et_lane = etab + lane * 8;

        auto load_e = [&](int h, T (&dst)[RPL]) {
            if constexpr (kETab) {
                const uint8_t* p = et_lane + (h << 9);
#pragma unroll
                for (int s2 = 0; s2 < RP2; ++s2) {
                    const float2 v = *reinterpret_cast<const float2*>(p + s2 * kNumCodes * 512);
                    dst[2 * s2] = v.x;
                    if (2 * s2 + 1 < RPL) dst[2 * s2 + 1] = v.y;
                }
            } else {
                const bool hN = (h == kCodeN);
#pragma unroll
                for (int s = 0; s < RPL; ++s) dst[s] = ((h == rb[s]) | hN) ? eM[s] : eX[s];
            }
        };

        const bool use_plain = EXACT || __any((int)zero_gap) != 0;
        constexpr int kPlain = 0, kScaled = 1, kSixOp = 2;

        auto sweep = [&](auto form_tag) {
            constexpr int FORM = decltype(form_tag)::value;
            constexpr bool SC = FORM == kScaled;
            constexpr bool SIX = FORM == kSixOp;
            T y_above = init_y;
            if constexpr (SC || SIX) {
                T g_own[RPL], g_below[RPL];
#pragma unroll
                for (int s = 0; s < RPL; ++s) g_own[s] = k1[s];
                T g_next_lane = shr1_down<G>(g_own[0]);
#pragma unroll
                for (int s = 0; s < RPL; ++s) g_below[s] = (s + 1 < RPL) ? g_own[s + 1] : g_next_lane;
                if (j == nl - 1) {
                    g_below[RPL - 1] = (T)1.0;
                    if constexpr (STRIP) { if (!last_strip) g_below[RPL - 1] = (T)1.0 - ph2pr[a.gcp[job.read_off + (uint64_t)(row_base + rows_here)] & 127]; }
                }
                T my_above[RPL];
                if constexpr (SIX) {
                    T my_own[RPL];
#pragma unroll
                    for (int s = 0; s < RPL; ++s) my_own[s] = clone[s] ? (T)1.0 : k4[s];
                    T my_top = (T)1.0;
                    if constexpr (STRIP) {
                        if (strip > 0) my_top = ph2pr[a.del[job.read_off + (uint64_t)(row_base - 1)] & 127];
                    }
                    my_above[0] = shr1<G>(my_top, my_own[RPL - 1]);
#pragma unroll
                    for (int s = 1; s < RPL; ++s) my_above[s] = my_own[s - 1];
                }
#pragma unroll
                for (int s = 0; s < RPL; ++s) {
                    if (clone[s]) {
                        py[s] = SIX ? init_y : g_below[s] * init_y;
                    } else {
                        const T gb = g_below[s];
                        const T pMX = k2[s], pXX = k3[s], pMY = k4[s];
                        k1[s] = gb * pMX;
                        k2[s] = gb * ratio[s];
                        if constexpr (SIX) k3[s] = g_own[s] * my_above[s];
                        else k3[s] = gb * pMY;
                        k4[s] = pXX;
                    }
                    if (clone[s]) { k1[s] = 0; k2[s] = 0; k3[s] = 0; k4[s] = 1; }
                }
                y_above = SIX ? init_y : g_own[0] * init_y;
            }
            const T old_y = (j == 0) ? y_above : (T)0;
            T uaM = 0, uaX = 0, uaY = old_y, ubM = 0, ubX = 0, ubY = old_y;
            if constexpr (STRIP) {
                if (strip > 0) {
                    uaY = 0; ubY = 0;
                    if (j == 0 && H > 0) { ubM = bprev[0]; ubX = bprev[a.strip_stride]; ubY = bprev[2u * a.strip_stride]; }
                }
            }

            auto column = [&](const T (&ec)[RPL], T& o2M, T& o2X, T& o2Y, const T o1M, const T o1X, bool count, const int dcol) {
                T Mn[RPL], Xn[RPL], Yn[RPL];
                if constexpr (SIX) {
                    Mn[0] = fma_(k3[0], o2Y, fma_(o2M, k0[0], o2X)) * ec[0];
                    Xn[0] = fma_(o1X, k2[0], o1M * k1[0]);
                    Yn[0] = fma_(py[0], k4[0], pm[0]);
#pragma unroll
                    for (int s = 1; s < RPL; ++s) {
                        Mn[s] = fma_(k3[s], py[s - 1], fma_(pm[s - 1], k0[s], px[s - 1])) * ec[s];
                        Xn[s] = fma_(Xn[s - 1], k2[s], Mn[s - 1] * k1[s]);
                        Yn[s] = fma_(py[s], k4[s], pm[s]);
                    }
                } else if constexpr (SC) {
                    Mn[0] = (fma_(o2M, k0[0], o2X) + o2Y) * ec[0];
                    Xn[0] = fma_(o1X, k2[0], o1M * k1[0]);
                    Yn[0] = fma_(py[0], k4[0], pm[0] * k3[0]);
#pragma unroll
                    for (int s = 1; s < RPL; ++s) {
                        Mn[s] = (fma_(pm[s - 1], k0[s], px[s - 1]) + py[s - 1]) * ec[s];
                        Xn[s] = fma_(Xn[s - 1], k2[s], Mn[s - 1] * k1[s]);
                        Yn[s] = fma_(py[s], k4[s], pm[s] * k3[s]);
                    }
                } else if constexpr (EXACT) {
                    Mn[0] = ((o2M * k0[0] + o2X * k1[0]) + o2Y * k1[0]) * ec[0];
                    Xn[0] = o1M * k2[0] + o1X * k3[0];
                    Yn[0] = pm[0] * k4[0] + py[0] * k3[0];
#pragma unroll
                    for (int s = 1; s < RPL; ++s) {
                        Mn[s] = ((pm[s - 1] * k0[s] + px[s - 1] * k1[s]) + py[s - 1] * k1[s]) * ec[s];
                        Xn[s] = Mn[s - 1] * k2[s] + Xn[s - 1] * k3[s];
                        Yn[s] = pm[s] * k4[s] + py[s] * k3[s];
                    }
                } else {
                    Mn[0] = fma_(o2Y, k1[0], fma_(o2X, k1[0], o2M * k0[0])) * ec[0];
                    Xn[0] = fma_(o1X, k3[0], o1M * k2[0]);
                    Yn[0] = fma_(py[0], k3[0], pm[0] * k4[0]);
#pragma unroll
                    for (int s = 1; s < RPL; ++s) {
                        Mn[s] = fma_(py[s - 1], k1[s], fma_(px[s - 1], k1[s], pm[s - 1] * k0[s])) * ec[s];
                        Xn[s] = fma_(Xn[s - 1], k3[s], Mn[s - 1] * k2[s]);
                        Yn[s] = fma_(py[s], k3[s], pm[s] * k4[s]);
                    }
                }
#pragma unroll
                for (int s = 0; s < RPL; ++s) { pm[s] = Mn[s]; px[s] = Xn[s]; py[s] = Yn[s]; }
                if (count && (!STRIP || last_strip)) { sumM += Mn[RPL - 1]; sumX += Xn[RPL - 1]; }
                o2M = shr1<G>(o2M, Mn[RPL - 1]);
                o2X = shr1<G>(o2X, Xn[RPL - 1]);
                o2Y = shr1<G>(o2Y, Yn[RPL - 1]);
                if constexpr (STRIP) {
                    if (strip > 0 && j == 0) {
                        const int c1 = dcol + 1;
                        const bool in = c1 < H;
                        o2M = in ? bprev[c1] : (T)0; o2X = in ? bprev[a.strip_stride + c1] : (T)0; o2Y = in ? bprev[2u * a.strip_stride + c1] : (T)0;
                    }
                    if (!last_strip && j == nl - 1) {
                        const int c = dcol - j;
                        if (c >= 0 && c < H) { bcur[c] = Mn[RPL - 1]; bcur[a.strip_stride + c] = Xn[RPL - 1]; bcur[2u * a.strip_stride + c] = Yn[RPL - 1]; }
                    }
                }
            };

            T e[RPL];
            int d = 0;
            int h1 = hp_lane[1];
            load_e((int)hp_lane[0], e);
            for (; d + 2 <= nmin; d += 2) {
                T e1[RPL];
                load_e(h1, e1);
                const int h2 = hp_lane[d + 2], h3 = hp_lane[d + 3];
                column(e, uaM, uaX, uaY, ubM, ubX, true, d);
                load_e(h2, e);
                column(e1, ubM, ubX, ubY, uaM, uaX, true, d + 1);
                h1 = h3;
            }
            for (; d < nmax; ++d) {
                const int hn = hp_lane[d + 1];
                column(e, uaM, uaX, uaY, ubM, ubX, d < nsteps_g, d);
                T t;
                t = uaM; uaM = ubM; ubM = t;
                t = uaX; uaX = ubX; ubX = t;
                t = uaY; uaY = ubY; ubY = t;
                load_e(hn, e);
            }
        };
        if constexpr (EXACT) sweep(std::integral_constant<int, kPlain>{});
        else if (use_plain) sweep(std::integral_constant<int, kPlain>{});
        else if constexpr (kSix) sweep(std::integral_constant<int, kSixOp>{});
        else sweep(std::integral_constant<int, kScaled>{});
      }

        if (live && j == nl - 1) {
            const T res = sumM + sumX;
            if constexpr (sizeof(T) == 4) {
                if (res < 1e-28f || group_hap_n) {
                    const uint32_t k = atomicAdd(a.rerun_count, 1u);
                    a.rerun_list[k] = job_idx;
                } else {
                    a.out_log10[job.pair] = (double)(log10f(res) - a.log10_initial_f);
                }
            } else {
                if (!EXACT && a.rerun_count && res < kExactBelow) {
                    const uint32_t k = atomicAdd(a.rerun_count, 1u);
                    a.rerun_list[k] = job_idx;
                } else {
                    a.out_log10[job.pair] = log10(res) - a.log10_initial_d;
                    a.used_f64[job.pair] = 1;
                }
            }
        }
    }
}

template <typename T, int G, int RPL>
#ifndef MGX_HMM_MINWAVES_8
#define MGX_HMM_MINWAVES_8 4
#endif
__global__ __launch_bounds__(256, (sizeof(T) == 4 && RPL == 7) ? MGX_HMM_MINWAVES_8 : (sizeof(T) == 4 && RPL == 10) ? 3 : 1) void pairhmm_fwd(KernelArgs a) {
    extern __shared__ __attribute__((aligned(16))) uint8_t smem[];
    pairhmm_body<T, G, RPL>(a, smem, blockIdx.x, gridDim.x);
}

constexpr int kStripG = 64, kStripRPL = 16;
template <typename T>
__global__ __launch_bounds__(64) void pairhmm_fwd_strip(KernelArgs a) {
    extern __shared__ __attribute__((aligned(16))) uint8_t smem[];
    pairhmm_body<T, kStripG, kStripRPL, true>(a, smem, blockIdx.x, gridDim.x);
}
__global__ __launch_bounds__(64) void pairhmm_fwd_exact(KernelArgs a) {
    extern __shared__ __attribute__((aligned(16))) uint8_t smem[];
    pairhmm_body<double, kStripG, kStripRPL, true, true>(a, smem, blockIdx.x, gridDim.x);
}

constexpr int kMultiBins = 16;
struct MultiArgs {
    KernelArgs a;
    uint32_t n_bins;
    uint32_t block_first[kMultiBins + 1];
    uint32_t job_first[kMultiBins], job_count[kMultiBins], lds_stride[kMultiBins];
    uint8_t G[kMultiBins], RPL[kMultiBins];
};

template <int GSET>
__device__ __forceinline__ void pairhmm_multi_body(const MultiArgs& m, uint8_t* smem) {
    uint32_t k = 0;
    while (k + 1 < m.n_bins && blockIdx.x >= m.block_first[k + 1]) ++k;
    KernelArgs a = m.a;
    a.job_first = m.job_first[k]; a.n_static = m.job_count[k]; a.lds_stride = m.lds_stride[k];
    const uint32_t blk = blockIdx.x - m.block_first[k], nblk = m.block_first[k + 1] - m.block_first[k];
    const int code = (int)m.G[k] * 16 + (int)m.RPL[k];
#define MGX_MCASE(g, r) case (g) * 16 + (r): pairhmm_body<float, g, r>(a, smem, blk, nblk); break;
    if constexpr (GSET == 0) {
        switch (code) {
            MGX_MCASE(16, 1) MGX_MCASE(16, 2) MGX_MCASE(16, 3) MGX_MCASE(16, 4) MGX_MCASE(16, 5) MGX_MCASE(16, 6) MGX_MCASE(16, 7) MGX_MCASE(16, 8)
            default: break;
        }
    } else {
        switch (code) {
            MGX_MCASE(8, 1) MGX_MCASE(8, 2) MGX_MCASE(8, 3) MGX_MCASE(8, 4) MGX_MCASE(8, 5) MGX_MCASE(8, 6) MGX_MCASE(8, 7) MGX_MCASE(8, 8)
            MGX_MCASE(4, 1) MGX_MCASE(4, 2) MGX_MCASE(4, 3) MGX_MCASE(4, 4) MGX_MCASE(4, 5) MGX_MCASE(4, 6) MGX_MCASE(4, 7) MGX_MCASE(4, 8)
            default: break;
        }
    }
#undef MGX_MCASE
}

template <int GSET>
__global__ __launch_bounds__(256) void pairhmm_fwd_multi(MultiArgs m) {
    extern __shared__ __attribute__((aligned(16))) uint8_t smem[];
    pairhmm_multi_body<GSET>(m, smem);
}

struct SeqRef {
    uint64_t off;
    uint32_t len;
    uint32_t id;
};

struct RegionRef {
    uint32_t hap_begin;
    uint32_t n_haps;
    uint32_t read_base;
    uint32_t out_base;
};
__global__ __launch_bounds__(256) void pairhmm_make_jobs_multi(const SeqRef* __restrict__ reads, const uint32_t* __restrict__ read_region,
                                                               const uint32_t* __restrict__ job_prefix, uint32_t n_reads,
                                                               const RegionRef* __restrict__ regions, const SeqRef* __restrict__ haps,
                                                               uint32_t n_jobs, Job* __restrict__ jobs) {
    const uint32_t q = blockIdx.x * 256 + threadIdx.x;
    if (q >= n_jobs) return;
    uint32_t lo = 0, hi = n_reads;
    while (hi - lo > 1) { const uint32_t m = lo + (hi - lo) / 2; if (job_prefix[m] <= q) lo = m; else hi = m; }
    const SeqRef r = reads[lo];
    const RegionRef g = regions[read_region[lo]];
    const SeqRef h = haps[g.hap_begin + (q - job_prefix[lo])];
    Job j;
    j.read_off = r.off; j.hap_off = h.off; j.R = r.len; j.H = h.len;
    j.pair = g.out_base + (r.id - g.read_base) * g.n_haps + h.id; j.pad_ = 0;
    jobs[q] = j;
}

struct ReadModel {
    uint8_t pcr_cache[21];
    int rate_factor;
    int bq_threshold;
    int constant_gcp;
};

__device__ __forceinline__ int n_repetitions(const uint8_t* s, int unit_off, int unit_len, int test_off, int test_len, bool leading) {
    if (test_len == 0) return 0;
    const int diff = test_len - unit_len;
    int n = 0;
    if (leading) {
        for (int st = 0; st <= diff; st += unit_len) {
            bool eq = true;
            for (int i = 0; i < unit_len; ++i) eq &= s[st + test_off + i] == s[unit_off + i];
            if (!eq) return n;
            ++n;
        }
    } else {
        for (int st = diff; st >= 0; st -= unit_len) {
            bool eq = true;
            for (int i = 0; i < unit_len; ++i) eq &= s[st + test_off + i] == s[unit_off + i];
            if (!eq) return n;
            ++n;
        }
    }
    return n;
}
__device__ int tandem_repeat_units(const uint8_t* b, int length, int offset) {
    int maxBW = 0, bw_off = offset, bw_len = 1;
    for (int str = 1; str <= 8; ++str) {
        if (offset + 1 - str < 0) break;
        maxBW = n_repetitions(b, offset - str + 1, str, 0, offset + 1, false);
        if (maxBW > 1) { bw_off = offset - str + 1; bw_len = str; break; }
    }
    int maxRL = maxBW;
    if (offset < length - 1) {
        int maxFW = 0, fw_len = 1;
        const int fw_off = offset + 1;
        for (int str = 1; str <= 8; ++str) {
            if (offset + str + 1 > length) break;
            maxFW = n_repetitions(b, offset + 1, str, offset + 1, length - offset - 1, true);
            if (maxFW > 1) { fw_len = str; break; }
        }
        bool same = fw_len == bw_len;
        if (same) for (int i = 0; i < fw_len; ++i) same &= b[fw_off + i] == b[bw_off + i];
        if (!same) maxBW = n_repetitions(b, fw_off, fw_len, 0, offset + 1, false);
        maxRL = maxFW + maxBW;
    }
    return maxRL > 20 ? 20 : maxRL;
}

__global__ __launch_bounds__(128) void pairhmm_read_model(const SeqRef* __restrict__ reads, const uint8_t* __restrict__ bases,
                                                          uint8_t* qual, uint8_t* ins, uint8_t* del, uint8_t* gcp,
                                                          const uint8_t* __restrict__ mapq, ReadModel m) {
    __shared__ uint8_t sb[1024 + 16];
    const SeqRef r = reads[blockIdx.x];
    const int len = (int)r.len;
    const bool in_lds = len <= 1024;
    if (in_lds) for (int i = threadIdx.x; i < len; i += blockDim.x) sb[i] = bases[r.off + i];
    __syncthreads();
    const uint8_t* sbp = in_lds ? sb : bases + r.off;
    const int mq = mapq[r.id];
    for (int i = threadIdx.x; i < len; i += blockDim.x) {
        int qi = ins[r.off + i], qd = del[r.off + i];
        if (m.rate_factor > 0 && i < len - 1) {
            const int c = m.pcr_cache[tandem_repeat_units(sbp, len, i)];
            qi = c < qi ? c : qi; qd = c < qd ? c : qd;
        }
        int q = qual[r.off + i];
        q = mq < q ? mq : q;
        qual[r.off + i] = (uint8_t)(q < m.bq_threshold ? 6 : q);
        ins[r.off + i] = (uint8_t)(qi < 6 ? 6 : qi);
        del[r.off + i] = (uint8_t)(qd < 6 ? 6 : qd);
        if (m.constant_gcp >= 0) gcp[r.off + i] = (uint8_t)m.constant_gcp;
    }
}

__global__ __launch_bounds__(256) void pairhmm_normalize_filter_rows(double* __restrict__ out, const uint64_t* __restrict__ read_len,
                                                                     const uint32_t* __restrict__ row_off, const uint32_t* __restrict__ row_nh,
                                                                     uint32_t n_reads, double log10_rate, double max_error_per_base,
                                                                     uint8_t* __restrict__ keep) {
    const uint32_t r = blockIdx.x * 4 + (threadIdx.x >> 6);
    const int lane = threadIdx.x & 63;
    if (r >= n_reads) return;
    const uint32_t n_haps = row_nh[r];
    double* row = out + row_off[r];
    double best = -__builtin_inf();
    for (uint32_t h = lane; h < n_haps; h += 64) best = fmax(best, row[h]);
#pragma unroll
    for (int off = 32; off > 0; off >>= 1) best = fmax(best, __shfl_xor(best, off, 64));
    if (!__builtin_isinf(log10_rate) && n_haps > 1) {
        const double cap = best + log10_rate;
        for (uint32_t h = lane; h < n_haps; h += 64) if (row[h] < cap) row[h] = cap;
    }
    if (lane == 0) {
        const double max_err = fmin(2.0, ceil((double)read_len[r] * max_error_per_base));
        keep[r] = !(best < max_err * -4.0);
    }
}

using KernelFn = void (*)(KernelArgs);

template <typename T>
KernelFn pick_kernel(int G, int RPL) {
#define MGX_CASE(g, r) if (G == g && RPL == r) return pairhmm_fwd<T, g, r>;
    MGX_CASE(4, 1) MGX_CASE(4, 2) MGX_CASE(4, 3) MGX_CASE(4, 4) MGX_CASE(4, 5) MGX_CASE(4, 6) MGX_CASE(4, 7) MGX_CASE(4, 8)
    MGX_CASE(8, 1) MGX_CASE(8, 2) MGX_CASE(8, 3) MGX_CASE(8, 4) MGX_CASE(8, 5) MGX_CASE(8, 6) MGX_CASE(8, 7) MGX_CASE(8, 8)
    MGX_CASE(16, 1) MGX_CASE(16, 2) MGX_CASE(16, 3) MGX_CASE(16, 4)
    MGX_CASE(16, 5) MGX_CASE(16, 6) MGX_CASE(16, 7) MGX_CASE(16, 8)
    if constexpr (sizeof(T) == 4) { MGX_CASE(16, 9) MGX_CASE(16, 10) MGX_CASE(16, 11) MGX_CASE(16, 12) }
    if constexpr (sizeof(T) == 8) { MGX_CASE(64, 3) }
    MGX_CASE(64, 4) MGX_CASE(64, 5) MGX_CASE(64, 6) MGX_CASE(64, 7) MGX_CASE(64, 8)
    MGX_CASE(64, 9) MGX_CASE(64, 10) MGX_CASE(64, 11) MGX_CASE(64, 12)
    MGX_CASE(64, 13) MGX_CASE(64, 14) MGX_CASE(64, 15) MGX_CASE(64, 16)
#undef MGX_CASE
    return nullptr;
}

}
```

Before: 6263.

## Split haplotypes by N content and route N-free jobs to four-code kernels

On the host, haplotypes in each region are split into N-free and N-containing views, and reads in selected shape classes (G16/G64 with RPL 7-8) get separate bin entries per view. N-free jobs run a 4-code fp32 kernel with a smaller per-wave emission table in LDS. N-containing jobs use the 5-code kernel, so the device-side N ballot and forced-rerun path are removed. The cost is more host planning (memchr per haplotype, extra region views and read entries), more kernel instantiations, and a new row_haps field to keep output indexing correct.

```diff
diff --git a/fast-genomic-data-processing_amd/csrc/mgx_pairhmm.hip b/fast-genomic-data-processing_amd/csrc/mgx_pairhmm.hip
--- a/fast-genomic-data-processing_amd/csrc/mgx_pairhmm.hip
+++ b/fast-genomic-data-processing_amd/csrc/mgx_pairhmm.hip
@@ -36,6 +36,7 @@
 
 struct Bin {
     int G = 0, RPL = 0;
+    int codes = 5;
     int Gd = 0, RPLd = 0;
     uint32_t job_begin = 0, job_count = 0;
     uint32_t max_h = 0;
@@ -139,22 +140,48 @@
 }
 inline uint32_t lds_bytes(const Bin& bin, bool f32) {
     const uint32_t waves = bin.block / 64u, groups = bin.block / (uint32_t)(f32 ? bin.G : bin.Gd);
-    const uint32_t etab = f32 ? (uint32_t)((bin.RPL + 1) / 2) * kNumCodes * 512u : 0u;
+    const uint32_t etab = f32 ? (uint32_t)((bin.RPL + 1) / 2) * (uint32_t)bin.codes * 512u : 0u;
     return waves * etab + groups * bin.lds_stride;
 }
-constexpr int kBinG8 = kNarrowMaxRPL, kBinG16 = kBinG8 + kG8MaxRPL, kBinG64 = kBinG16 + kG16MaxRPL;
-constexpr int kBinStrip = kBinG64 + (kG64MaxRPL - kG64MinRPL + 1);
-constexpr int kBins = kBinStrip + 1;
-inline int bin_index(int G, int RPL) {
-    if (G == 64 && RPL == kStripMarkRPL) return kBinStrip;
-    return G == 4 ? RPL - 1 : G == 8 ? kBinG8 + RPL - 1 : G == 16 ? kBinG16 + RPL - 1 : kBinG64 + RPL - kG64MinRPL;
-}
-inline void bin_shape(int k, Bin* b) {
-    if (k == kBinStrip) { b->G = 64; b->RPL = kG64MaxRPL; b->Gd = 64; b->RPLd = kG64MaxRPL; b->strip = true; return; }
-    if (k < kBinG8) { b->G = 4; b->RPL = k + 1; }
-    else if (k < kBinG16) { b->G = 8; b->RPL = k - kBinG8 + 1; }
-    else if (k < kBinG64) { b->G = 16; b->RPL = k - kBinG16 + 1; }
-    else { b->G = 64; b->RPL = k - kBinG64 + kG64MinRPL; }
+constexpr int kClassG8 = kNarrowMaxRPL, kClassG16 = kClassG8 + kG8MaxRPL, kClassG64 = kClassG16 + kG16MaxRPL;
+constexpr int kClassStrip = kClassG64 + (kG64MaxRPL - kG64MinRPL + 1);
+constexpr int kClasses = kClassStrip + 1;
+inline int class_index(int G, int RPL) {
+    if (G == 64 && RPL == kStripMarkRPL) return kClassStrip;
+    return G == 4 ? RPL - 1 : G == 8 ? kClassG8 + RPL - 1 : G == 16 ? kClassG16 + RPL - 1 : kClassG64 + RPL - kG64MinRPL;
+}
+inline bool four_code_class(int k) {
+    return k == kClassG16 + 6 || k == kClassG16 + 7 || k == kClassG64 + 7 - kG64MinRPL || k == kClassG64 + 8 - kG64MinRPL;
+}
+constexpr int kBins = kClasses + 4;
+struct BinSlot { int cls; int codes; };
+struct BinTable { BinSlot slot[kBins]; int first[kClasses]; };
+inline const BinTable& bin_table() {
+    static const BinTable table = [] {
+        BinTable t{};
+        int at = 0;
+        for (int k = 0; k < kClasses; ++k) {
+            t.first[k] = at;
+            if (four_code_class(k)) t.slot[at++] = BinSlot{k, 4};
+            t.slot[at++] = BinSlot{k, 5};
+        }
+        return t;
+    }();
+    return table;
+}
+inline const BinSlot* bin_slots() { return bin_table().slot; }
+inline int bin_index(int cls, bool hap_n) { return bin_table().first[cls] + (four_code_class(cls) && hap_n); }
+inline void class_shape(int k, int* G, int* RPL) {
+    if (k < kClassG8) { *G = 4; *RPL = k + 1; }
+    else if (k < kClassG16) { *G = 8; *RPL = k - kClassG8 + 1; }
+    else if (k < kClassG64) { *G = 16; *RPL = k - kClassG16 + 1; }
+    else { *G = 64; *RPL = k == kClassStrip ? kG64MaxRPL : k - kClassG64 + kG64MinRPL; }
+}
+inline void bin_shape(int slot, Bin* b) {
+    const BinSlot sl = bin_slots()[slot];
+    b->codes = sl.codes;
+    class_shape(sl.cls, &b->G, &b->RPL);
+    if (sl.cls == kClassStrip) { b->Gd = 64; b->RPLd = kG64MaxRPL; b->strip = true; return; }
     if (b->G == 16 && b->RPL > 8) { b->Gd = 64; b->RPLd = (16 * b->RPL + 63) / 64; }
     else { b->Gd = b->G; b->RPLd = b->RPL; }
 }
@@ -164,8 +191,10 @@
     bin.lds_stride = (bin.max_h + 2u * (uint32_t)std::max(bin.G, bin.Gd) + 8u + 15u) & ~15u;
     bin.block = 64;
     if (const char* e = getenv("MGX_PAIRHMM_BLOCK")) { const int v = atoi(e); if (v == 64 || v == 128 || v == 256) bin.block = (uint32_t)v; }
-    while (bin.block > 64u && lds_bytes(bin, true) > kMaxLdsPerBlock) bin.block /= 2;
-    if (lds_bytes(bin, true) > 160u * 1024u) {
+    Bin five = bin;
+    five.codes = 5;
+    while (bin.block > 64u && lds_bytes(five, true) > kMaxLdsPerBlock) five.block = bin.block /= 2;
+    if (lds_bytes(five, true) > 160u * 1024u) {
         set_error("haplotype of %u bases does not fit the LDS staging buffer", bin.max_h);
         return -E2BIG;
     }
@@ -181,15 +210,21 @@
     return 0;
 }
 void merge_small_bins(uint64_t (&count)[kBins], int (&remap)[kBins]) {
+    const BinSlot* sl = bin_slots();
     for (int k = 0; k < kBins; ++k) remap[k] = k;
     for (int k = 0; k + 1 < kBins; ++k) {
-        if (k + 1 == kBinG8 || k + 1 == kBinG16 || k + 1 == kBinG64 || k + 1 == kBinStrip) continue;
-        if (count[k] && count[k] < kMergeBelow) { count[k + 1] += count[k]; count[k] = 0; remap[k] = k + 1; }
+        const int t = sl[k + 1].codes == 4 ? k + 2 : k + 1;
+        int G, Gt, RPL;
+        class_shape(sl[k].cls, &G, &RPL); class_shape(sl[t].cls, &Gt, &RPL);
+        if (G != Gt || sl[t].cls == kClassStrip) continue;
+        if (count[k] && count[k] < kMergeBelow) { count[t] += count[k]; count[k] = 0; remap[k] = t; }
     }
     for (int k = 0; k < kBins; ++k) { int t = k; while (remap[t] != t) t = remap[t]; remap[k] = t; }
 }
 
 inline size_t align_up(size_t x, size_t a = 256) { return (x + a - 1) / a * a; }
+
+inline bool hap_has_n(const uint8_t* hap, uint64_t len) { return memchr(hap, 'N', len) != nullptr; }
 
 int acquire_slab(mgx_pairhmm* c, size_t bytes, size_t pin_bytes, Slab* out) {
     int best = -1;
@@ -341,6 +376,7 @@
 
 struct SlabLayout {
     uint64_t n = 0, n_reads = 0, n_haps = 0, n_regions = 0, read_bytes = 0, hap_bytes = 0;
+    uint64_t n_entries = 0;
     bool cross = false, model = false;
     size_t rtab = 0, rreg = 0, rpre = 0, gtab = 0, htab = 0;
     size_t jobs = 0, bases = 0, qual = 0, ins = 0, del = 0, gcp = 0, hap = 0;
@@ -355,9 +391,9 @@
     auto take = [&off](size_t bytes) { const size_t at = off; off = align_up(off + bytes); return at; };
     const uint64_t n = L->n, per_read = L->model ? L->n_reads : 0;
     if (L->cross) {
-        L->rtab = take(L->n_reads * sizeof(SeqRef));
-        L->rreg = take(L->n_reads * sizeof(uint32_t));
-        L->rpre = take((L->n_reads + 1) * sizeof(uint32_t));
+        L->rtab = take(L->n_entries * sizeof(SeqRef));
+        L->rreg = take(L->n_entries * sizeof(uint32_t));
+        L->rpre = take((L->n_entries + 1) * sizeof(uint32_t));
         L->gtab = take(L->n_regions * sizeof(RegionRef));
         L->htab = take(L->n_haps * sizeof(SeqRef));
     } else {
@@ -409,15 +445,26 @@
     return rm;
 }
 
-struct CrossRead { uint64_t off; uint32_t len, region; uint8_t bin; };
+struct CrossRead { uint64_t off; uint32_t len, region; uint8_t bin, bin_n; };
+struct CrossEntry { uint8_t bin; uint32_t view; };
 struct CrossPlan {
     uint64_t nr = 0, nh = 0, n = 0, read_bytes = 0, hap_bytes = 0;
     std::vector<CrossRead> reads;
     std::vector<RegionRef> regions;
     std::vector<SeqRef> haps;
+    std::vector<uint64_t> sum_h;
     uint32_t max_h = 0;
+    uint64_t n_entries = 0;
     uint64_t reads_in[kBins] = {0}, rstart[kBins + 1] = {0}, jobs_in[kBins] = {0}, cells_in[kBins] = {0}, bytes_in[kBins] = {0};
 };
+
+inline int cross_entries(const CrossPlan& p, const CrossRead& ri, CrossEntry (&e)[2]) {
+    const uint32_t v = 3u * ri.region;
+    if (ri.bin == ri.bin_n || !p.regions[v + 2].n_haps) { e[0] = CrossEntry{ri.bin, v}; return 1; }
+    if (!p.regions[v + 1].n_haps) { e[0] = CrossEntry{ri.bin_n, v}; return 1; }
+    e[0] = CrossEntry{ri.bin, v + 1}; e[1] = CrossEntry{ri.bin_n, v + 2};
+    return 2;
+}
 
 int cross_totals(uint32_t n_regions, const mgx_pairhmm_input_t* regs, CrossPlan* p, std::vector<uint64_t>* out_base) {
     out_base->assign(n_regions + 1, 0);
@@ -435,33 +482,60 @@
 
 int cross_tables(uint32_t n_regions, const mgx_pairhmm_input_t* regs, const std::vector<uint64_t>& out_base, CrossPlan* p,
                  uint64_t (&count)[kBins]) {
-    p->reads.resize(p->nr); p->regions.resize(n_regions); p->haps.resize(p->nh);
-    uint64_t r_at = 0, h_at = 0, rb = 0, hb = 0;
+    p->reads.resize(p->nr); p->regions.resize(3 * (size_t)n_regions); p->sum_h.assign(3 * (size_t)n_regions, 0);
+    p->haps.clear(); p->haps.reserve(p->nh);
+    uint64_t r_at = 0, rb = 0, hb = 0;
+    std::vector<uint8_t> with_n;
     for (uint32_t g = 0; g < n_regions; ++g) {
         const mgx_pairhmm_input_t& in = regs[g];
-        RegionRef& R = p->regions[g];
-        R.hap_begin = (uint32_t)h_at; R.n_haps = (uint32_t)in.n_haps; R.read_base = (uint32_t)r_at; R.out_base = (uint32_t)out_base[g];
-        for (uint64_t h = 0; h < in.n_haps; ++h) {
-            const uint64_t H = in.hap_off[h + 1] - in.hap_off[h];
-            if (H == 0) { set_error("region %u: haplotype %llu is empty", g, (unsigned long long)h); return -EINVAL; }
-            if (H > 0x7FFFFFF0ull) { set_error("haplotype too long"); return -E2BIG; }
-            p->haps[h_at + h] = SeqRef{hb + (in.hap_off[h] - in.hap_off[0]), (uint32_t)H, (uint32_t)h};
-            p->max_h = std::max<uint32_t>(p->max_h, (uint32_t)H);
-        }
-        std::stable_sort(p->haps.begin() + h_at, p->haps.begin() + h_at + in.n_haps, [](const SeqRef& a, const SeqRef& b2) { return a.len > b2.len; });
+        bool any_four = false;
         for (uint64_t r = 0; r < in.n_reads; ++r) {
             const uint64_t Rl = in.read_off[r + 1] - in.read_off[r];
             if (Rl == 0) { set_error("region %u: read %llu is empty", g, (unsigned long long)r); return -EINVAL; }
             int G, RPL;
             shape_of((uint32_t)std::min<uint64_t>(Rl, 0xFFFFFFFFull), &G, &RPL);
             if (G == 0) { set_error("region %u: read of %llu bases exceeds the %d-row limit", g, (unsigned long long)Rl, kMaxRowsStrip); return -E2BIG; }
+            const int cls = class_index(G, RPL);
             CrossRead& ri = p->reads[r_at + r];
-            ri.off = rb + (in.read_off[r] - in.read_off[0]); ri.len = (uint32_t)Rl; ri.region = g; ri.bin = (uint8_t)bin_index(G, RPL);
-            count[ri.bin] += in.n_haps;
+            ri.off = rb + (in.read_off[r] - in.read_off[0]); ri.len = (uint32_t)Rl; ri.region = g;
+            ri.bin = (uint8_t)bin_index(cls, false); ri.bin_n = (uint8_t)bin_index(cls, true);
+            any_four |= four_code_class(cls);
+        }
+        const size_t h_at = p->haps.size();
+        with_n.assign(in.n_haps, 0);
+        for (uint64_t h = 0; h < in.n_haps; ++h) {
+            const uint64_t H = in.hap_off[h + 1] - in.hap_off[h];
+            if (H == 0) { set_error("region %u: haplotype %llu is empty", g, (unsigned long long)h); return -EINVAL; }
+            if (H > 0x7FFFFFF0ull) { set_error("haplotype too long"); return -E2BIG; }
+            p->haps.push_back(SeqRef{hb + (in.hap_off[h] - in.hap_off[0]), (uint32_t)H, (uint32_t)h});
+            p->max_h = std::max<uint32_t>(p->max_h, (uint32_t)H);
+            if (any_four) with_n[h] = hap_has_n(in.hap_bases + in.hap_off[h], H);
+        }
+        std::stable_sort(p->haps.begin() + h_at, p->haps.end(), [](const SeqRef& a, const SeqRef& b2) { return a.len > b2.len; });
+        uint32_t n_kind[2] = {0, 0};
+        uint64_t sum_kind[2] = {0, 0};
+        for (uint64_t h = 0; h < in.n_haps; ++h) { const SeqRef& hr = p->haps[h_at + h]; n_kind[with_n[hr.id]]++; sum_kind[with_n[hr.id]] += hr.len; }
+        RegionRef all;
+        all.hap_begin = (uint32_t)h_at; all.n_haps = (uint32_t)in.n_haps; all.read_base = (uint32_t)r_at; all.out_base = (uint32_t)out_base[g];
+        all.row_haps = (uint32_t)in.n_haps;
+        RegionRef kind[2] = {all, all};
+        if (n_kind[0] && n_kind[1]) {
+            kind[0].hap_begin = (uint32_t)p->haps.size(); kind[0].n_haps = n_kind[0];
+            for (uint64_t h = 0; h < in.n_haps; ++h) { const SeqRef hr = p->haps[h_at + h]; if (!with_n[hr.id]) p->haps.push_back(hr); }
+            kind[1].hap_begin = (uint32_t)p->haps.size(); kind[1].n_haps = n_kind[1];
+            for (uint64_t h = 0; h < in.n_haps; ++h) { const SeqRef hr = p->haps[h_at + h]; if (with_n[hr.id]) p->haps.push_back(hr); }
+        } else {
+            kind[n_kind[0] ? 1 : 0].n_haps = 0;
+        }
+        p->regions[3 * (size_t)g] = all; p->regions[3 * (size_t)g + 1] = kind[0]; p->regions[3 * (size_t)g + 2] = kind[1];
+        p->sum_h[3 * (size_t)g] = sum_kind[0] + sum_kind[1]; p->sum_h[3 * (size_t)g + 1] = sum_kind[0]; p->sum_h[3 * (size_t)g + 2] = sum_kind[1];
+        for (uint64_t r = 0; r < in.n_reads; ++r) {
+            const CrossRead& ri = p->reads[r_at + r];
+            count[ri.bin] += n_kind[0]; count[ri.bin_n] += n_kind[1];
         }
         if (in.n_reads) rb += in.read_off[in.n_reads] - in.read_off[0];
         if (in.n_haps) hb += in.hap_off[in.n_haps] - in.hap_off[0];
-        r_at += in.n_reads; h_at += in.n_haps;
+        r_at += in.n_reads;
     }
     return 0;
 }
@@ -469,14 +543,16 @@
 void cross_bins(CrossPlan* p, uint64_t (&count)[kBins]) {
     int remap[kBins];
     merge_small_bins(count, remap);
-    std::vector<uint64_t> sumH(p->regions.size(), 0);
-    for (size_t g = 0; g < p->regions.size(); ++g)
-        for (uint32_t h = 0; h < p->regions[g].n_haps; ++h) sumH[g] += p->haps[p->regions[g].hap_begin + h].len;
     for (CrossRead& ri : p->reads) {
-        ri.bin = (uint8_t)remap[ri.bin];
-        const RegionRef& R = p->regions[ri.region];
-        p->reads_in[ri.bin]++; p->jobs_in[ri.bin] += R.n_haps; p->cells_in[ri.bin] += (uint64_t)ri.len * sumH[ri.region];
-        p->bytes_in[ri.bin] += 5ull * ri.len * R.n_haps + sumH[ri.region] + 4ull * R.n_haps;
+        ri.bin = (uint8_t)remap[ri.bin]; ri.bin_n = (uint8_t)remap[ri.bin_n];
+        CrossEntry e[2];
+        const int ne = cross_entries(*p, ri, e);
+        for (int q = 0; q < ne; ++q) {
+            const uint64_t nh = p->regions[e[q].view].n_haps, sum = p->sum_h[e[q].view];
+            p->reads_in[e[q].bin]++; p->jobs_in[e[q].bin] += nh; p->cells_in[e[q].bin] += (uint64_t)ri.len * sum;
+            p->bytes_in[e[q].bin] += 5ull * ri.len * nh + sum + 4ull * nh;
+        }
+        p->n_entries += (uint64_t)ne;
     }
     for (int k = 0; k < kBins; ++k) p->rstart[k + 1] = p->rstart[k] + p->reads_in[k];
 }
@@ -489,15 +565,19 @@
     for (int k = 0; k < kBins; ++k) cur[k] = p.rstart[k];
     for (uint64_t r = 0; r < p.nr; ++r) {
         const CrossRead& ri = p.reads[r];
-        const uint64_t at = cur[ri.bin]++;
-        rtab[at] = SeqRef{ri.off, ri.len, (uint32_t)r};
-        rreg[at] = ri.region;
+        CrossEntry e[2];
+        const int ne = cross_entries(p, ri, e);
+        for (int q = 0; q < ne; ++q) {
+            const uint64_t at = cur[e[q].bin]++;
+            rtab[at] = SeqRef{ri.off, ri.len, (uint32_t)r};
+            rreg[at] = e[q].view;
+        }
     }
     uint32_t run = 0;
-    for (uint64_t at = 0; at < p.nr; ++at) { rpre[at] = run; run += p.regions[rreg[at]].n_haps; }
-    rpre[p.nr] = run;
-    memcpy(pin + L.gtab, p.regions.data(), n_regions * sizeof(RegionRef));
-    memcpy(pin + L.htab, p.haps.data(), p.nh * sizeof(SeqRef));
+    for (uint64_t at = 0; at < p.n_entries; ++at) { rpre[at] = run; run += p.regions[rreg[at]].n_haps; }
+    rpre[p.n_entries] = run;
+    memcpy(pin + L.gtab, p.regions.data(), p.regions.size() * sizeof(RegionRef));
+    memcpy(pin + L.htab, p.haps.data(), p.haps.size() * sizeof(SeqRef));
     size_t rb = 0, hb = 0;
     for (uint32_t g = 0; g < n_regions; ++g) {
         const mgx_pairhmm_input_t& in = regs[g];
@@ -548,7 +628,8 @@
     if ((rc = cross_tables(n_regions, regs, *out_base, &p, count))) return rc;
     cross_bins(&p, count);
     SlabLayout L;
-    L.n = p.n; L.n_reads = p.nr; L.n_haps = p.nh; L.n_regions = n_regions; L.read_bytes = p.read_bytes; L.hap_bytes = p.hap_bytes;
+    L.n = p.n; L.n_reads = p.nr; L.n_entries = p.n_entries; L.n_haps = p.haps.size(); L.n_regions = p.regions.size();
+    L.read_bytes = p.read_bytes; L.hap_bytes = p.hap_bytes;
     L.cross = true; L.model = model != nullptr;
     if ((rc = lay_out_slab(c, true, &L, b))) return rc;
     uint8_t* dv = b->slab.dev; uint8_t* pin = b->slab.pin;
@@ -561,7 +642,7 @@
     }
     HIP_TRY(hipMemcpyAsync(dv, pin, b->in_bytes, hipMemcpyHostToDevice, s));
     if (model)
-        hipLaunchKernelGGL(pairhmm_read_model, dim3((uint32_t)p.nr), dim3(128), 0, s, (const SeqRef*)(dv + L.rtab),
+        hipLaunchKernelGGL(pairhmm_read_model, dim3((uint32_t)p.n_entries), dim3(128), 0, s, (const SeqRef*)(dv + L.rtab), (const uint32_t*)(dv + L.rreg),
                            b->d_bases, b->d_qual, b->d_ins, b->d_del, b->d_gcp, (const uint8_t*)(dv + L.mapq), make_read_model(*model));
     uint64_t job_begin = 0;
     for (int k = 0; k < kBins; ++k) {
@@ -579,7 +660,7 @@
         job_begin += bin.job_count;
     }
     hipLaunchKernelGGL(pairhmm_make_jobs_multi, dim3((uint32_t)((p.n + 255) / 256)), dim3(256), 0, s, (const SeqRef*)(dv + L.rtab),
-                       (const uint32_t*)(dv + L.rreg), (const uint32_t*)(dv + L.rpre), (uint32_t)p.nr, (const RegionRef*)(dv + L.gtab),
+                       (const uint32_t*)(dv + L.rreg), (const uint32_t*)(dv + L.rpre), (uint32_t)p.n_entries, (const RegionRef*)(dv + L.gtab),
                        (const SeqRef*)(dv + L.htab), (uint32_t)p.n, b->d_jobs);
     HIP_TRY(hipGetLastError());
     HIP_TRY(hipEventCreateWithFlags(&b->uploaded, hipEventDisableTiming));
@@ -639,6 +720,11 @@
     std::vector<uint32_t> bin_of(n);
     uint64_t count[kBins] = {0};
     uint32_t max_h = 0;
+    std::vector<int8_t> hap_n(n_haps, -1);
+    auto has_n = [&](uint32_t h) {
+        if (hap_n[h] < 0) hap_n[h] = hap_has_n(in->hap_bases + (plan ? in->hap_off[plan->lhap[h]] : hoff[h]), hoff[h + 1] - hoff[h]);
+        return hap_n[h] != 0;
+    };
     for (uint64_t i = 0; i < n; ++i) {
         const uint32_t r = pr[i], h = ph[i];
         if (r >= n_reads || h >= n_haps) { set_error("test case %llu: index out of range", (unsigned long long)i); return -EINVAL; }
@@ -649,7 +735,8 @@
         shape_of((uint32_t)std::min<uint64_t>(R, 0xFFFFFFFFull), &G, &RPL);
         if (G == 0) { set_error("test case %llu: read of %llu bases exceeds the %d-row limit", (unsigned long long)i, (unsigned long long)R, kMaxRowsStrip); return -E2BIG; }
         if (H > 0x7FFFFFF0ull) { set_error("haplotype too long"); return -E2BIG; }
-        const int bi = bin_index(G, RPL);
+        const int cls = class_index(G, RPL);
+        const int bi = bin_index(cls, four_code_class(cls) && has_n(h));
         bin_of[i] = (uint32_t)bi;
         count[bi]++;
         max_h = std::max<uint32_t>(max_h, (uint32_t)H);
@@ -829,7 +916,9 @@
         m.block_first[q] = blocks; blocks += bn.grid_f32;
         m.job_first[q] = bn.job_begin; m.job_count[q] = bn.job_count; m.lds_stride[q] = bn.lds_stride;
         m.G[q] = (uint8_t)bn.G; m.RPL[q] = (uint8_t)bn.RPL;
-        lds = std::max(lds, lds_bytes(bn, true));
+        Bin five = bn;
+        five.codes = 5;
+        lds = std::max(lds, lds_bytes(five, true));
         if (bn.cells > b->bins[book].cells) book = set[q];
         cells += bn.cells; bytes += bn.alg_bytes;
         r.in_multi[set[q]] = 1;
@@ -883,8 +972,8 @@
     if (!r.force_f64 && !r.in_multi[k]) {
         a.job_list = nullptr; a.n_dyn = nullptr; a.n_static = bin.job_count;
         a.ph2pr = c->d_ph2pr_f; a.mm = c->d_mm_f; a.ph2pr_div3 = c->d_div3_f; a.gap_ratio = c->d_ratio_f;
-        KernelFn f = bin.strip ? (KernelFn)pairhmm_fwd_strip<float> : pick_kernel<float>(bin.G, bin.RPL);
-        if (!f) { set_error("no fp32 kernel for G=%d RPL=%d", bin.G, bin.RPL); return -ENOSYS; }
+        KernelFn f = bin.strip ? (KernelFn)pairhmm_fwd_strip<float> : pick_kernel<float>(bin.G, bin.RPL, bin.codes);
+        if (!f) { set_error("no fp32 kernel for G=%d RPL=%d with %d codes", bin.G, bin.RPL, bin.codes); return -ENOSYS; }
         if (r.timing) HIP_TRY(hipEventRecord(ev[4 * k + 0], sk));
         hipLaunchKernelGGL(f, dim3(bin.grid_f32), dim3(bin.block), lds_bytes(bin, true), sk, a);
         if (r.timing) HIP_TRY(hipEventRecord(ev[4 * k + 1], sk));
@@ -1038,7 +1127,7 @@
             st.dominant_cells = cells_of(dom);
             st.dominant_alg_bytes = acct ? b->acct_bytes[dom] : b->bins[dom].alg_bytes;
             if (acct && b->acct_multi[dom]) snprintf(st.dominant_kernel, sizeof st.dominant_kernel, "pairhmm_fwd_multi<%d>", b->acct_multi[dom] - 1);
-            else snprintf(st.dominant_kernel, sizeof st.dominant_kernel, "pairhmm_fwd<float, %d, %d>", b->bins[dom].G, b->bins[dom].RPL);
+            else snprintf(st.dominant_kernel, sizeof st.dominant_kernel, "pairhmm_fwd<float, %d, %d, %d>", b->bins[dom].G, b->bins[dom].RPL, b->bins[dom].codes);
         }
         b->runs_timed = 0;
     }
diff --git a/fast-genomic-data-processing_amd/csrc/pairhmm_kernels.hip.inc b/fast-genomic-data-processing_amd/csrc/pairhmm_kernels.hip.inc
--- a/fast-genomic-data-processing_amd/csrc/pairhmm_kernels.hip.inc
+++ b/fast-genomic-data-processing_amd/csrc/pairhmm_kernels.hip.inc
@@ -104,16 +104,13 @@
     static __device__ __forceinline__ double initial() { return 0x1p1020; }
 };
 
-#ifndef MGX_PAIRHMM_CODES
-#define MGX_PAIRHMM_CODES 5
-#endif
-constexpr int kNumCodes = MGX_PAIRHMM_CODES;
-template <int RPL> constexpr int etab_bytes_per_wave() { return ((RPL + 1) / 2) * kNumCodes * 64 * 8; }
-
-template <typename T, int G, int RPL, bool STRIP = false, bool EXACT = false>
+template <int RPL, int CODES> constexpr int etab_bytes_per_wave() { return ((RPL + 1) / 2) * CODES * 64 * 8; }
+
+template <typename T, int G, int RPL, bool STRIP = false, bool EXACT = false, int CODES = 5>
 __device__ __forceinline__ void pairhmm_body(const KernelArgs& a, uint8_t* smem, const uint32_t block, const uint32_t n_blocks) {
     constexpr int GPW = 64 / G;
     constexpr bool kETab = (sizeof(T) == 4);
+    static_assert(CODES == 5 || (CODES == 4 && kETab), "four codes: the fp32 emission table only");
     constexpr bool kSix = (sizeof(T) == 4) && !EXACT;
     constexpr int RP2 = (RPL + 1) / 2;
     constexpr int S = lane_stride<G>();
@@ -124,8 +121,8 @@
     const int j = G < 16 ? (lane & 15) / S : lane % G;
     const int grp = wave * GPW + (G < 16 ? (lane >> 4) * S + (lane & 15) % S : lane / G);
     const int n_waves = (int)blockDim.x >> 6;
-    uint8_t* etab = smem + (kETab ? (size_t)wave * etab_bytes_per_wave<RPL>() : 0);
-    uint8_t* hapbuf = smem + (kETab ? (size_t)n_waves * etab_bytes_per_wave<RPL>() : 0) +
+    uint8_t* etab = smem + (kETab ? (size_t)wave * etab_bytes_per_wave<RPL, CODES>() : 0);
+    uint8_t* hapbuf = smem + (kETab ? (size_t)n_waves * etab_bytes_per_wave<RPL, CODES>() : 0) +
                       (size_t)grp * a.lds_stride;
     const T* __restrict__ ph2pr = (const T*)a.ph2pr;
     const T* __restrict__ mm = (const T*)a.mm;
@@ -149,7 +146,6 @@
         const int first_rows = R - (n_strips - 1) * kStripRows;
 
         __syncthreads();
-        bool hap_n = false;
         {
             const uint8_t* hp = a.hap_bases + job.hap_off;
             const int n_words = (int)a.lds_stride >> 2;
@@ -166,27 +162,13 @@
 #pragma unroll
                     for (int t = 0; t < 4; ++t) {
                         const int c = c0 + t;
-                        const int code = (live && c >= 0 && c < H) ? base_code(hp[c]) : (kNumCodes > 4 ? kCodeN : 0);
+                        const int code = (live && c >= 0 && c < H) ? base_code(hp[c]) : (CODES > 4 ? kCodeN : 0);
                         packed |= (uint32_t)code << (8 * t);
                     }
                 }
-                if constexpr (kETab && kNumCodes == 4) {
-                    const uint32_t x = packed ^ (0x01010101u * (uint32_t)kCodeN);
-                    hap_n |= ((x - 0x01010101u) & ~x & 0x80808080u) != 0;
-                    packed &= 0x03030303u;
-                }
                 hb32[w] = packed;
             }
         }
-        bool group_hap_n = false;
-        if constexpr (kETab && kNumCodes == 4) {
-            uint64_t gmask;
-            if constexpr (G == 64) gmask = ~0ull;
-            else if constexpr (G == 16) gmask = 0xFFFFull << (lane & 48);
-            else gmask = (uint64_t)((G == 8 ? 0x5555u : 0x1111u) << ((lane & 15) % S)) << (lane & 48);
-            group_hap_n = (__ballot((int)hap_n) & gmask) != 0;
-        }
-
         T sumM = 0, sumX = 0;
         bool zero_gap = false;
         if constexpr (STRIP) {
@@ -245,8 +227,8 @@
 #pragma unroll
             for (int s = 0; s < RPL; ++s)
 #pragma unroll
-                for (int code = 0; code < kNumCodes; ++code)
-                    et[((s >> 1) * kNumCodes + code) * 128 + (s & 1)] =
+                for (int code = 0; code < CODES; ++code)
+                    et[((s >> 1) * CODES + code) * 128 + (s & 1)] =
                         (code == rb[s] || code == kCodeN) ? eM[s] : eX[s];
         }
         __syncthreads();
@@ -274,7 +256,7 @@
                 const uint8_t* p = et_lane + (h << 9);
 #pragma unroll
                 for (int s2 = 0; s2 < RP2; ++s2) {
-                    const float2 v = *reinterpret_cast<const float2*>(p + s2 * kNumCodes * 512);
+                    const float2 v = *reinterpret_cast<const float2*>(p + s2 * CODES * 512);
                     dst[2 * s2] = v.x;
                     if (2 * s2 + 1 < RPL) dst[2 * s2 + 1] = v.y;
                 }
@@ -437,7 +419,7 @@
         if (live && j == nl - 1) {
             const T res = sumM + sumX;
             if constexpr (sizeof(T) == 4) {
-                if (res < 1e-28f || group_hap_n) {
+                if (res < 1e-28f) {
                     const uint32_t k = atomicAdd(a.rerun_count, 1u);
                     a.rerun_list[k] = job_idx;
                 } else {
@@ -456,13 +438,13 @@
     }
 }
 
-template <typename T, int G, int RPL>
+template <typename T, int G, int RPL, int CODES = 5>
 #ifndef MGX_HMM_MINWAVES_8
 #define MGX_HMM_MINWAVES_8 4
 #endif
 __global__ __launch_bounds__(256, (sizeof(T) == 4 && RPL == 7) ? MGX_HMM_MINWAVES_8 : (sizeof(T) == 4 && RPL == 10) ? 3 : 1) void pairhmm_fwd(KernelArgs a) {
     extern __shared__ __attribute__((aligned(16))) uint8_t smem[];
-    pairhmm_body<T, G, RPL>(a, smem, blockIdx.x, gridDim.x);
+    pairhmm_body<T, G, RPL, false, false, CODES>(a, smem, blockIdx.x, gridDim.x);
 }
 
 constexpr int kStripG = 64, kStripRPL = 16;
@@ -526,6 +508,7 @@
     uint32_t n_haps;
     uint32_t read_base;
     uint32_t out_base;
+    uint32_t row_haps;
 };
 __global__ __launch_bounds__(256) void pairhmm_make_jobs_multi(const SeqRef* __restrict__ reads, const uint32_t* __restrict__ read_region,
                                                                const uint32_t* __restrict__ job_prefix, uint32_t n_reads,
@@ -540,7 +523,7 @@
     const SeqRef h = haps[g.hap_begin + (q - job_prefix[lo])];
     Job j;
     j.read_off = r.off; j.hap_off = h.off; j.R = r.len; j.H = h.len;
-    j.pair = g.out_base + (r.id - g.read_base) * g.n_haps + h.id; j.pad_ = 0;
+    j.pair = g.out_base + (r.id - g.read_base) * g.row_haps + h.id; j.pad_ = 0;
     jobs[q] = j;
 }
 
@@ -596,10 +579,12 @@
     return maxRL > 20 ? 20 : maxRL;
 }
 
-__global__ __launch_bounds__(128) void pairhmm_read_model(const SeqRef* __restrict__ reads, const uint8_t* __restrict__ bases,
+__global__ __launch_bounds__(128) void pairhmm_read_model(const SeqRef* __restrict__ reads, const uint32_t* __restrict__ read_view,
+                                                          const uint8_t* __restrict__ bases,
                                                           uint8_t* qual, uint8_t* ins, uint8_t* del, uint8_t* gcp,
                                                           const uint8_t* __restrict__ mapq, ReadModel m) {
     __shared__ uint8_t sb[1024 + 16];
+    if (read_view[blockIdx.x] % 3u == 2u) return;
     const SeqRef r = reads[blockIdx.x];
     const int len = (int)r.len;
     const bool in_lds = len <= 1024;
@@ -648,7 +633,16 @@
 using KernelFn = void (*)(KernelArgs);
 
 template <typename T>
-KernelFn pick_kernel(int G, int RPL) {
+KernelFn pick_kernel(int G, int RPL, int codes = 5) {
+    if constexpr (sizeof(T) == 4) {
+        if (codes == 4) {
+            if (G == 16 && RPL == 7) return pairhmm_fwd<T, 16, 7, 4>;
+            if (G == 16 && RPL == 8) return pairhmm_fwd<T, 16, 8, 4>;
+            if (G == 64 && RPL == 7) return pairhmm_fwd<T, 64, 7, 4>;
+            if (G == 64 && RPL == 8) return pairhmm_fwd<T, 64, 8, 4>;
+            return nullptr;
+        }
+    }
 #define MGX_CASE(g, r) if (G == g && RPL == r) return pairhmm_fwd<T, g, r>;
     MGX_CASE(4, 1) MGX_CASE(4, 2) MGX_CASE(4, 3) MGX_CASE(4, 4) MGX_CASE(4, 5) MGX_CASE(4, 6) MGX_CASE(4, 7) MGX_CASE(4, 8)
     MGX_CASE(8, 1) MGX_CASE(8, 2) MGX_CASE(8, 3) MGX_CASE(8, 4) MGX_CASE(8, 5) MGX_CASE(8, 6) MGX_CASE(8, 7) MGX_CASE(8, 8)
```

New measurement: 6475 (median of 6 runs). 1.03x the previous value.
